# TruongKhang/cds-mvsnet

Measured on AMD Instinct MI355X. Metric: depth-maps/sec per ref view at 640x512 N=5 D=192 (single-stage plane sweep incl. CostRegNet + regression), higher is better.
Workload: dtype f32; 1 GPU; M1: single-stage StageNet volume 640x512, D=192, C=8, N=5 views; parallelism=single

## Files before the change

### cds_mvsnet_amd/_lib.py

```python
from __future__ import annotations

import ctypes
import os
from ctypes import c_float, c_int, c_longlong, c_void_p

_HERE = os.path.dirname(os.path.abspath(__file__))
LIB_PATH = os.environ.get("CDS_MVSNET_LIB") or os.path.join(_HERE, "libcdsmvs_hip.so")

ACT_NONE, ACT_RELU, ACT_LEAKY01, ACT_SIGMOID, ACT_TANH = 0, 1, 2, 3, 4
ACT_ACCUM = 16
AGG_ACCUMULATE, AGG_NORMALIZE, AGG_CHANNELS_LAST, AGG_FAST_POSITIONS = 1, 2, 4, 8
WARP_FAST_POSITIONS = AGG_FAST_POSITIONS
MAX_VIEWS = 8
MAX_IMAGES = 16
STAGE_STATE_WORDS = 2080
DEPTH_METRICS_MAX_T = 8
DEPTH_METRICS_MAX_GROUPS = 1024
ICP_SUMS = 18
ICP_MAX_GROUPS = 1024
CROP_MAX_VERTICES = 256
RANSAC_RECORD = 15
RANSAC_MIN_SAMPLE, RANSAC_MAX_SAMPLE = 3, 8
EINVAL = -1000

P = c_void_p
I = c_int
F = c_float
DB = ctypes.c_double
L = c_longlong

SIGNATURES = {
    "cds_version": [],
    "cds_chw_to_hwc_f32": [P, P, I, I, I, P],
    "cds_stage_inputs_f32": [P, P, P, P, P, P, P, P, P, P, I, I, I, I, P],
    "cds_homo_warp_f32": [P, P, P, P, I, I, I, I, I, P],
    "cds_warp_entropy_f32": [P, P, P, P, P, I, I, I, I, I, I, P],
    "cds_warp_entropy_flags_f32": [P, P, P, P, P, I, I, I, I, I, I, I, P],
    "cds_warp_aggregate_f32": [P, P, P, P, P, P, P, I, I, I, I, I, I, I, P],
    "cds_warp_entropy_window_f32": [P, P, P, P, P, I, I, I, I, I, I, I, I, P],
    "cds_warp_aggregate_window_f32": [P, P, P, P, P, P, P, I, I, I, I, I, I, I, I, P],
    "cds_warp_aggregate_bwd_f32": [P, P, P, P, P, P, P, P, P, I, I, I, I, I, I, P],
    "cds_volume_finish_f32": [P, P, P, I, I, I, I, P, P, P],
    "cds_volume_finish_bwd_f32": [P, P, P, P, P, I, I, I, I, P, P, P, P, P],
    "cds_volume_normalize_f32": [P, P, I, I, I, P],
    "cds_volume_normalize_cl_f32": [P, P, I, I, I, P],
    "cds_softargmin_conf_f32": [P, P, P, P, P, I, I, I, I, P],
    "cds_depth_hypotheses_f32": [P, P, I, I, I, I, I, I, P, P, P],
    "cds_depth_planes_f32": [P, I, I, I, P, P],
    "cds_conv3d_k3_f32": [P, P, P, P, P, I, I, I, I, I, I, I, P],
    "cds_conv3d_k3_cl_f32": [P, P, P, P, P, I, I, I, I, I, I, P],
    "cds_conv3d_sbf_f32": [P, P, P, P, P, I, I, I, I, I, I, I, P],
    "cds_conv3d_sf16_f32": [P, P, P, P, I, I, I, I, I, I, I, P, F, P, P],
    "cds_deconv3d_sbf_f32": [P, P, P, P, P, I, I, I, I, I, I, I, P],
    "cds_deconv3d_sf16_f32": [P, P, P, P, P, I, I, I, I, I, I, P, F, P, P],
    "cds_deconv3d_zm_sf16_f32": [P, P, P, P, P, I, I, I, I, I, I, P, F, P, P],
    "cds_deconv_prob_zm_f32": [P, P, P, P, P, P, I, I, I, P],
    "cds_deconv_prob_zm_sf16_f32": [P, P, P, P, P, P, I, I, I, P, F, P],
    "cds_deconv_prob_zm_sf16_mfma_f32": [P, P, P, P, P, P, P, I, I, I, P, F, P, F, F, P],
    "cds_deconv3d_zm_f32": [P, P, P, P, P, I, I, I, I, I, I, P],
    "cds_deconv3d_k3s2_f32": [P, P, P, P, P, I, I, I, I, I, I, P],
    "cds_conv2d_f32": [P, P, P, P, I, I, I, I, I, I, I, I, I, P],
    "cds_conv2d_affine_f32": [P, P, P, P, P, I, I, I, I, I, I, I, I, I, P],
    "cds_instnorm_affine_f32": [P, P, P, I, I, I, I, F, P],
    "cds_fpn_stats_parts": [I, I],
    "cds_conv2d_fpn_f32": [P, P, P, P, P, P, P, I, I, I, I, I, I, P],
    "cds_conv2d_k3_c16_f32": [P, P, P, P, P, P, I, I, I, I, P],
    "cds_dynconv_branches_sbf_f32": [P, P, P, P, P, I, I, I, I, I, P, I, P],
    "cds_dynconv_fused_sbf_f32": [P, P, P, P, P, P, P, P, F, P, P, P, I, I, I, I, I, P, I, P],
    "cds_dynconv_fused_parts": [I, I],
    "cds_conv2d_k3_relu_sbf_f32": [P, P, P, P, P, P, I, I, I, I, P],
    "cds_dynconv_blend_f32": [P, P, P, P, P, F, P, P, I, I, I, I, I, P],
    "cds_dynconv_blend_shared_f32": [P, P, P, P, P, F, P, P, I, I, I, I, I, I, P],
    "cds_blend_stats_parts": [I, I],
    "cds_dynconv_blend_stats_f32": [P, P, P, P, P, F, P, P, P, I, I, I, I, I, I, P],
    "cds_instnorm_reduce_f32": [P, I, P, P, I, I, I, I, F, P],
    "cds_instnorm_apply_f32": [P, P, P, I, I, I, I, I, I, P],
    "cds_instnorm_act_f32": [P, P, P, I, I, I, I, I, I, P],
    "cds_debug_poison_lds": [ctypes.c_uint],
    "cds_dynconv_cl_parts": [I, I],
    "cds_dynconv_cl_f32": [P, P, P, P, P, P, P, P, F, P, P, P, I, I, I, I, P, I, P],
    "cds_dynconv_cl_sf16_f32": [P, P, P, P, P, P, P, P, F, P, P, P, I, I, I, I, P, I, F, F, P],
    "cds_conv00_cl_f32": [P, P, P, P, P, P, P, F, P, P, P, I, I, I, I, P],
    "cds_conv00_cl_sf16_f32": [P, P, P, P, P, P, P, F, P, P, P, I, I, I, I, P, F, P],
    "cds_blend_cl_parts": [I, I],
    "cds_dynconv_blend_cl_f32": [P, P, P, P, P, F, P, P, P, I, I, I, I, I, I, P],
    "cds_conv2d_k3s2_cl_f32": [P, P, P, P, I, I, I, I, I, P],
    "cds_conv2d_k3s2_cl_sf16_f32": [P, P, P, P, I, I, I, I, I, F, F, P],
    "cds_fpn_cl_parts": [I, I],
    "cds_conv2d_fpn_cl_f32": [P, P, P, P, P, P, P, I, I, I, I, I, I, P],
    "cds_vis_layer1_cl_f32": [P, P, P, P, P, I, I, I, P],
    "cds_conv2d_k3_relu_cl_f32": [P, P, P, P, P, P, I, I, I, I, P],
    "cds_vis_cnn_rm_f32": [P, P, P, P, P, P, P, P, P, P, P, I, I, I, P],
    "cds_instnorm_stats_cl_parts": [I, I],
    "cds_instnorm_stats_cl_f32": [P, P, I, I, I, I, P],
    "cds_instnorm_apply_cl_f32": [P, P, P, P, I, I, I, I, I, I, I, P],
    "cds_curvature_stats_f32": [P, P, P, P, P, I, P],
    "cds_curvature_stats_bwd_f32": [P, P, P, P, P, P, P, P, I, P],
    "cds_pair_mean_f32": [P, P, I, I, P],
    "cds_view_mean_f32": [P, P, I, I, P],
    "cds_depth_affine_f32": [P, P, I, P, P],
    "cds_deconv2d_k3s2_f32": [P, P, P, P, I, I, I, I, I, P],
    "cds_refine_finish_f32": [P, P, P, I, I, P, P],
    "cds_bn3d_stats_f32": [P, P, I, I, L, P],
    "cds_bn3d_norm_f32": [P, P, P, P, DB, DB, F, P, P, P, P, P, P, P, P, I, I, L, I, P],
    "cds_bn3d_bwd_reduce_f32": [P, P, P, P, P, I, I, L, I, P],
    "cds_bn3d_bwd_norm_f32": [P, P, P, P, P, P, P, DB, P, P, P, I, I, L, I, P],
    "cds_conv3d_wgrad_f32": [P, P, P, I, I, I, I, I, I, I, I, I, I, P],
    "cds_bn3d_norm_bound_f32": [P, P, P, P, DB, DB, F, P, P, P, P, P, P, P, P, I, I, L, I, P, P],
    "cds_bn3d_bwd_norm_bound_f32": [P, P, P, P, P, P, P, DB, P, P, P, I, I, L, I, P, P],
    "cds_absmax_bound_f32": [P, L, P, P],
    "cds_sf16_pack_conv3d_f32": [P, P, P, P, I, I, I, P],
    "cds_conv3d_k3_sf16_f32": [P, P, P, P, P, I, I, I, I, I, I, I, P],
    "cds_conv3d_wgrad_sf16_f32": [P, P, P, P, P, I, I, I, I, I, I, I, I, I, I, P],
    "cds_conv2d_wgrad_f32": [P, P, P, I, I, I, I, I, I, I, I, I, I, P],
    "cds_conv2d_dgrad_s2_f32": [P, P, P, I, I, I, I, I, I, I, P],
    "cds_instnorm_bwd_f32": [P, P, P, P, P, I, I, I, I, I, I, P],
    "cds_dynconv_bn_stats_f32": [P, P, P, P, P, P, P, P, I, I, I, I, I, I, F, F, I, I, P],
    "cds_dynconv_blend_train_f32": [P, P, P, P, P, P, P, P, F, P, P, I, I, I, I, I, I, P],
    "cds_dynconv_blend_bwd_f32": [P, P, P, P, P, P, P, P, F, P, P, P, P, P, I, I, I, I, I, I, I, I, P],
    "cds_f32_to_bf16": [P, P, L, P],
    "cds_instnorm_act_b16_f32": [P, P, P, P, P, I, I, I, I, I, I, P],
    "cds_conv2d_wgrad_xb16_f32": [P, P, P, I, I, I, I, I, I, I, I, I, I, P],
    "cds_instnorm_bwd_yb16_f32": [P, P, P, P, P, P, I, I, I, I, I, I, P],
    "cds_dynconv_bn_stats_b16_f32": [P, P, P, P, P, P, P, P, I, I, I, I, I, I, F, F, I, I, P],
    "cds_dynconv_blend_train_b16_f32": [P, P, P, P, P, P, P, P, F, P, P, I, I, I, I, I, I, P],
    "cds_dynconv_blend_bwd_b16_f32": [P, P, P, P, P, P, P, P, F, P, P, P, P, P, I, I, I, I, I, I, I, I, P],
    "cds_pack_conv2d_f32": [P, P, P, P, I, I, I, I, P],
    "cds_pack_conv3d_f32": [P, P, P, I, I, I, P],
    "cds_softargmin_bwd_f32": [P, P, P, P, I, I, I, I, P],
    "cds_dynconv_bwd_finish_f32": [P, P, I, I, P, P],
    "cds_bn_running_update_f32": [P, P, P, F, I, I, P, P, P],
    "cds_loss_records": [ctypes.c_longlong],
    "cds_loss_stage_f32": [P, P, P, P, P, P, P, I, I, I, P, P, P],
    "cds_loss_final_f32": [P, P, P, P, P, P, I, P, P, P, P],
    "cds_loss_stage_bwd_f32": [P, P, P, P, P, P, P, P, F, I, I, I, P, P, P, P],
    "cds_feat_target_f32": [P, P, P, F, F, I, I, I, P, P],
    "cds_depth_fusion_f32": [P, P, P, P, P, P, P, P, P, I, I, I, P, F, F, F, P],
    "cds_depth_fusion_dynamic_f32": [P, P, P, P, P, P, P, P, P, P, I, I, I, P, F, F, I, I, P],
    "cds_depth_normals_f32": [P, P, P, I, I, I, F, I, P, P, P],
    "cds_voxel_merge_f32": [P, P, P, L, P, P, L, P, P, P, P, P],
    "cds_tsdf_integrate_f32": [P, L, P, P, DB, P, P, P, P, I, I, I, P, P, P, P, P],
    "cds_tsdf_integrate_w_f32": [P, L, P, P, DB, P, P, P, P, I, I, I, P, P, P, P, P, I, F, P, P],
    "cds_tsdf_view_weights": [P, P, P, P, P, P, I, I, P, P],
    "cds_tsdf_classify": [P, P, L, P, P, P, P, I, P, P, P, P, P],
    "cds_tsdf_emit": [P, P, L, P, P, P, P, P, P, P, P, P, P, L, L, P, P, P, P, P],
    "cds_raster_project": [P, L, P, I, P, P, P],
    "cds_raster_faces": [P, L, L, P, I, P, P, I, I, L, P, P, P],
    "cds_raster_large": [P, L, P, L, L, P, I, P, P, I, I, P, P],
    "cds_raster_resolve": [P, P, L, L, P, I, P, P, I, I, P, P, P, P, P, P],
    "cds_mesh_cc_init": [P, L, P],
    "cds_mesh_cc_hook": [P, L, L, P, P, P],
    "cds_mesh_cc_jump": [P, L, P],
    "cds_mesh_cc_count": [P, L, L, P, P, P],
    "cds_mesh_cc_mark": [P, L, L, P, P, P, P, P],
    "cds_mesh_cc_gather": [P, P, P, L, L, P, P, P, P, L, L, P, P, P, P],
    "cds_mesh_simplify_faces": [P, L, L, P, L, P, P, P, P],
    "cds_mesh_simplify_quadric_f32": [P, L, P, L, P, P, P, P, L, F, P, P, P],
    "cds_mesh_simplify_mark": [P, P, L, L, P, P],
    "cds_mesh_simplify_gather": [P, P, L, P, P, P, L, P, P, L, L, P, P, P, P],
    "cds_mesh_adj_small": [],
    "cds_mesh_adj_count": [P, L, L, P, P],
    "cds_mesh_adj_fill": [P, L, L, P, P, P, L, P],
    "cds_mesh_adj_finish": [L, P, P, L, P, P, P],
    "cds_mesh_smooth_step_f32": [P, P, L, P, P, P, DB, P],
    "cds_mesh_smooth_limit_f32": [P, P, L, DB, P, P, P],
    "cds_mesh_fill_max_edges": [],
    "cds_mesh_fill_keys": [P, L, L, P, P],
    "cds_mesh_fill_borders": [P, L, L, P, P, P, P, P],
    "cds_mesh_fill_init": [L, P, P, P, P, P, P, P, P, P, P],
    "cds_mesh_fill_double": [P, L, L, P, P, P, P, P],
    "cds_mesh_fill_walk": [P, P, L, P, P, P, P, L, I, P, P, P, P],
    "cds_mesh_fill_emit": [P, P, L, L, P, L, I, P, P, P, P, P, L, L, P, P, P, P],
    "cds_mesh_sample_max_n": [],
    "cds_mesh_sample_count": [P, L, P, L, DB, P, P, P],
    "cds_mesh_sample_emit": [P, P, L, P, L, P, P, L, P, P, P, P],
    "cds_texture_votes": [P, P, I, I, I, L, P, I, P],
    "cds_texture_best": [P, L, I, I, P, P],
    "cds_texture_cells": [P, L, P, L, P, I, P, L, DB, I, P, P, P],
    "cds_texture_place": [P, P, L, L, I, P, P, P],
    "cds_texture_fill": [P, P, L, P, L, P, P, L, P, I, P, P, P, P, L, I, I, I, P, I, P],
    "cds_texture_level_samples": [P, L, P, P, L, P, I, P, L, P, P, P],
    "cds_texture_level_pairs": [P, P, P, P, L, I, P, P],
    "cds_texture_level_step": [P, P, P, P, P, L, P, L, L, I, DB, P, P, P],
    "cds_texture_fill_level": [P, P, L, P, L, P, P, L, P, I, P, P, P, P, L, I, I, I, P, I, P, P, L, P],
    "cds_photo_shade": [P, L, P, L, P, P, I, I, P, I, P, I, I, P, P],
    "cds_photo_scores": [P, P, P, P, I, I, I, P, L, P, P, P, P],
    "cds_grid_hash_log2_slots": [L],
    "cds_grid_keys_f32": [P, L, P, P, P],
    "cds_grid_hash_build": [P, L, L, P, P, I, P],
    "cds_nn_query_f32": [P, P, L, P, P, P, P, P, P, I, P, F, P, P],
    "cds_thin_round_f32": [P, P, L, P, P, I, P, F, P, P, P],
    "cds_knn_mean_f64": [P, P, L, P, P, P, P, P, P, I, P, I, F, P, P, P],
    "cds_knn_mean_wg_f64": [P, P, L, P, P, P, P, P, P, I, P, I, F, P, P, I, P],
    "cds_radius_count_f32": [P, P, L, P, P, P, P, P, P, I, P, F, I, P, P],
    "cds_outlier_stats_f64": [P, L, P, L, P, P],
    "cds_transform_points_f32": [P, L, P, P, P],
    "cds_nn_index_f32": [P, P, L, P, P, P, P, P, P, I, P, F, P, P, P],
    "cds_icp_sums_f64": [P, P, L, P, P, P, P, P, P, P, I, P, F, P, L, P, P, P, P],
    "cds_voxel_mean_f32": [P, L, P, P, L, P, P],
    "cds_polygon_crop_f32": [P, L, P, I, I, DB, DB, P, P],
    "cds_ransac_similarity_f64": [P, P, L, L, I, DB, ctypes.c_ulonglong, P, L, P, P, P, P],
    "cds_gipuma_tiles": [L],
    "cds_gipuma_prob_filter_f32": [P, P, P, I, I, I, P, P, P, P],
    "cds_gipuma_fuse_view_f32": [P, P, P, P, I, I, I, I, F, F, F, I, P, P, P, P],
    "cds_gipuma_scan": [P, I, P, P, P, P],
    "cds_gipuma_compact_f32": [P, P, P, I, I, P, P, P, P],
    "cds_colmap_score_quantum_log2": [],
    "cds_colmap_score_limbs": [DB, DB, DB],
    "cds_colmap_pair_scores_f64": [P, P, P, P, P, P, L, L, I, DB, DB, DB, I, P, P],
    "cds_colmap_obs_depth_f64": [P, P, P, P, L, P, P],
    "cds_colmap_depth_ranges_f64": [P, P, P, P, I, P, P],
    "cds_depth_metrics_f32": [P, P, P, P, F, I, L, I, P, L, P, P],
    "cds_gt_pyramid_f32": [P, P, I, I, I, P, P, I, I, I, P, P, P],
    "cds_image_batch_u8": [P, I, I, I, P, P, I, I, P, P],
    "cds_eval_views_u8": [P, I, I, I, P, P, P, P, P, P, I, I, P, P],
    "cds_eval_outputs_f32": [P, I, I, P, I, I, P, I, I, P, I, I, P, I, I, P, P, P],
}

_lib = None


class CdsLibraryError(RuntimeError):
    pass


def load() -> ctypes.CDLL:
    global _lib
    if _lib is not None:
        return _lib
    if not os.path.exists(LIB_PATH):
        raise CdsLibraryError(
            f"{LIB_PATH} not found: build it with `make -C {os.path.join(_HERE, 'csrc')}` "
            "(or `python -c 'import __graft_entry__ as g; g.build()'`). "
            "cds_mvsnet_amd has no CPU / PyTorch fallback.")
    import torch

    lib = ctypes.CDLL(LIB_PATH)
    for name, argtypes in SIGNATURES.items():
        try:
            fn = getattr(lib, name)
        except AttributeError as e:
            raise CdsLibraryError(f"{LIB_PATH} does not export {name}") from e
        fn.argtypes = argtypes
        fn.restype = c_int
    _lib = lib
    return lib


def check(rc: int, what: str) -> None:
    if rc == 0:
        return
    if rc == EINVAL:
        raise ValueError(f"{what}: invalid argument (CDS_EINVAL)")
    raise RuntimeError(f"{what}: HIP error {-rc}")
```

### cds_mvsnet_amd/csrc/conv3d_zmg.hip

```cpp
#include <stdlib.h>

#include "cds_common.hpp"
#include "sbf_common.hpp"

namespace {

__device__ __attribute__((aligned(32))) float g_zmg_zeros[8];

struct ZGDefaults {
  static constexpr int S = 1, RD = 1, MB = 1, TXO = 16, TYO = 8, G = 1, NG = 1, CW = 8, RPW = 1, YS = 1, PF = 1;
  static constexpr bool PAIR = false, F16 = false, P32 = false;
};
template <class P>
struct ZgF16 : P {
  static constexpr bool F16 = true;
};

struct ZgPair8 : ZGDefaults {
  static constexpr bool PAIR = true;
  static constexpr int TXO = 32, G = 3;
};
struct ZgPair16 : ZGDefaults {
  static constexpr bool PAIR = true;
  static constexpr int RD = 2, TXO = 32, NG = 4, CW = 4;
};
struct ZgPair32 : ZGDefaults {
  static constexpr bool PAIR = true;
  static constexpr int RD = 4, TXO = 32, TYO = 3, NG = 3, CW = 4;
};
struct ZgConv1 : ZGDefaults {
  static constexpr int S = 2;
};
struct ZgConv2 : ZGDefaults {
  static constexpr int RD = 2, TXO = 32;
};
struct ZgConv3 : ZGDefaults {
  static constexpr int S = 2, RD = 2, MB = 2, TYO = 4;
};
struct ZgConv2F16 : ZgF16<ZgConv2> {
  static constexpr int RPW = 2;
  static constexpr bool P32 = true;
};
struct ZgConv3F16 : ZgF16<ZgConv3> {
  static constexpr int RPW = 2;
};
struct ZgConv4F16 : ZgF16<ZGDefaults> {
  static constexpr int RD = 4, MB = 2, TYO = 4, PF = 2;
};
struct ZgConv5F16 : ZgF16<ZGDefaults> {
  static constexpr int S = 2, RD = 4, MB = 4, TYO = 2, RPW = 2;
  static constexpr bool P32 = true;
};
struct ZgConv6F16 : ZgF16<ZGDefaults> {
  static constexpr int RD = 8, MB = 4, TYO = 2, RPW = 2, YS = 2;
};

template <class P>
struct ZG {
  static constexpr int S = P::S, RD = P::RD, MB = P::MB, TXO = P::TXO, TYO = P::TYO, G = P::G, NG = P::NG;
  static constexpr bool F16 = P::F16;
  static constexpr int NT = F16 ? 2 : 3;
  static constexpr bool PAIR = P::PAIR, DEINT = PAIR || S == 2;
  static constexpr int CW = P::CW, PW = 4, THREADS = (CW + PW) * 64;
  static constexpr int RPW = P::RPW, YS = P::YS, PF = P::PF;
  static_assert(PF == 1 || (PF == 2 && 2 * NG * NT <= 15), "operand prefetch distance (lgkmcnt is a 4-bit count)");
  static_assert(RD % RPW == 0 && MB % YS == 0, "rounds per wave / cout split");
  static constexpr int KSPL = RD / RPW, MBS = MB / YS;
  static_assert(CW % (KSPL * MBS) == 0 && (KSPL == 1 || KSPL == 2 || KSPL == 4), "consumer waves");
  static constexpr int PARTS = CW / (KSPL * MBS);
  static constexpr int ROWS = TYO / PARTS;
  static constexpr int XT = TXO / (PAIR ? 32 : 16);
  static constexpr int NTW = ROWS * XT * G;
  static_assert(TYO % PARTS == 0 && NTW % NG == 0 && (KSPL != 2 || NTW % 2 == 0), "tile split");
  static constexpr int KW = PAIR ? 4 : 3, KS = (9 * KW + 3) / 4;
  static constexpr int IX = (TXO - 1) * S + 3, IY = (TYO - 1) * S + 3;
  static constexpr int IXH = DEINT ? (IX + 1) / 2 : 0;
  static constexpr int IXP = DEINT ? 2 * IXH : IX;
  static constexpr bool P32 = P::P32;
  static_assert(!P32 || F16, "the 32-byte position holds two terms");
  static constexpr int PB = P32 ? 16 : POSB, TB = P32 ? IY * IXP * 16 : 16;
  static constexpr int SLICEB = IY * IXP * (P32 ? 32 : POSB), PLANEB = RD * SLICEB;
  static constexpr int NINIT = 3 - S;
  static constexpr int NRES = S * (G - 1) + 3, NNEW = S * G, R = NRES + NNEW;
  static constexpr int RINGB = R * PLANEB;
  static constexpr int XCH1 = KSPL == 2 ? CW * (NTW / 2) * 1024 : (KSPL == 4 ? CW * NTW * 1024 : 0);
  static constexpr int NFIN = KSPL == 4 ? (NTW + 3) / 4 : 1;
  static constexpr int tap_of(int t, int gg) {
    const int tap = PAIR ? 4 * t + ((gg & 1) * 2 + (gg >> 1)) : 4 * t + gg;
    return tap > 9 * KW - 1 ? 9 * KW - 1 : tap;
  }
  static constexpr int tap_kz(int t, int gg) { return tap_of(t, gg) / (3 * KW); }
  static constexpr int tap_off(int t, int gg) {
    const int tap = tap_of(t, gg), ky = (tap / KW) % 3, kx = tap % KW;
    return (ky * IXP + (DEINT ? ((kx & 1) * IXH + (kx >> 1)) : kx)) * PB;
  }
  static constexpr int LDSB = RINGB + 2 * XCH1;
  static_assert(LDSB <= 160 * 1024, "LDS budget");
  static constexpr int NITEM = NNEW * IY * RD * IXP;
  static constexpr int PT = PW * 64, PPT = (NITEM + PT - 1) / PT;
};

template <class Cfg>
__global__ __launch_bounds__(Cfg::THREADS, 1) void conv3d_zmg_kernel(const float* __restrict__ x, const uint4* __restrict__ wsp,
                                                                  const float* __restrict__ bias, float* __restrict__ out, int Cout,
                                                                  int D, int H, int W, int Do, int Ho, int Wo, int act,
                                                                  int tiles_x, int tiles_y, int zseg,
                                                                  const float* __restrict__ in_bound, float w_inv,
                                                                  float* __restrict__ out_bound) {
  constexpr int S = Cfg::S, RD = Cfg::RD, G = Cfg::G, R = Cfg::R, Cin = 8 * RD, KS = Cfg::KS, NTW = Cfg::NTW, NG = Cfg::NG;
  constexpr bool PAIR = Cfg::PAIR, F16 = Cfg::F16;
  constexpr int NT = Cfg::NT;
  const float xs = F16 ? sf16_scale(in_bound[0]) : 1.0f;
  const float out_mul = F16 ? w_inv / xs : 1.0f;
  extern __shared__ __attribute__((aligned(16))) unsigned char lds[];
  const int tid = threadIdx.x;
  const int lane = tid & 63;
  const int wave = __builtin_amdgcn_readfirstlane(tid >> 6);
  const int nseg = (Do + zseg - 1) / zseg;
  int unit = cds_xcd_remap(blockIdx.x, gridDim.x);
  const int seg = unit % nseg;
  unit /= nseg;
  const int tx_i = unit % tiles_x, ty_i = unit / tiles_x;
  const int z0 = seg * zseg, z1 = min(Do, z0 + zseg);
  const int nstages = (z1 - z0 + G - 1) / G;
  const int gx0 = tx_i * Cfg::TXO * S - 1, gy0 = ty_i * Cfg::TYO * S - 1;
  const int zin0 = S * z0 - 1;

  if (wave >= Cfg::CW) {
#ifndef CDS_ZMG_PPRIO
#define CDS_ZMG_PPRIO 3
#endif
    __builtin_amdgcn_s_setprio(CDS_ZMG_PPRIO);
    constexpr int PT = Cfg::PT, PPT = Cfg::PPT;
    const int ptid = tid - Cfg::CW * 64;
    int s_pl[PPT], s_dst[PPT];
    long long s_off[PPT];
    unsigned okmask = 0;
#pragma unroll
    for (int h = 0; h < PPT; ++h) {
      const int p = h * PT + ptid;
      const int q = p % Cfg::IXP, t1 = p / Cfg::IXP;
      const int rd = t1 % RD, t2 = t1 / RD;
      const int row = t2 % Cfg::IY, pl = t2 / Cfg::IY;
      const int c = Cfg::DEINT ? (2 * (q % Cfg::IXH) + q / Cfg::IXH) : q;
      const int gy = gy0 + row, gx = gx0 + c;
      const bool exists = p < Cfg::NITEM && c < Cfg::IX;
      s_pl[h] = pl;
      s_dst[h] = rd * Cfg::SLICEB + (row * Cfg::IXP + q) * Cfg::PB;
      s_off[h] = ((long long)gy * W + gx) * Cin + rd * 8;
      if (exists && (unsigned)gy < (unsigned)H && (unsigned)gx < (unsigned)W) okmask |= 1u << h;
      if (!exists) s_pl[h] = -1;
    }
    const long long plane_elems = (long long)H * W * Cin;
    float4 va[2][PPT], vb[2][PPT];
    auto issue = [&](int st, int set) {
      const int zn = zin0 + st * S * G + Cfg::NINIT;
#pragma unroll
      for (int h = 0; h < PPT; ++h) {
        const int z = zn + s_pl[h];
        const bool ok = ((okmask >> h) & 1u) && (unsigned)z < (unsigned)D;
        const float* __restrict__ src = ok ? x + ((long long)z * plane_elems + s_off[h]) : g_zmg_zeros;
        va[set][h] = *reinterpret_cast<const float4*>(src);
        vb[set][h] = *reinterpret_cast<const float4*>(src + 4);
      }
    };
    auto deposit = [&](int st, int set) {
      const int slot0 = (st * S * G + Cfg::NINIT) % R;
#pragma unroll
      for (int h = 0; h < PPT; ++h) {
        if (h + 1 == PPT && s_pl[h] < 0) continue;
        int slot = slot0 + (s_pl[h] < 0 ? 0 : s_pl[h]);
        slot = slot >= R ? slot - R : slot;
        if (Cfg::P32) split_store8_f16_planar(lds + slot * Cfg::PLANEB + s_dst[h], Cfg::TB, va[set][h], vb[set][h], xs);
        else if (F16) split_store8_f16(lds + slot * Cfg::PLANEB + s_dst[h], va[set][h], vb[set][h], xs);
        else split_store8(lds + slot * Cfg::PLANEB + s_dst[h], va[set][h], vb[set][h]);
      }
    };
    for (int p = ptid; p < Cfg::NINIT * Cfg::IY * RD * Cfg::IXP; p += PT) {
      const int q = p % Cfg::IXP, t1 = p / Cfg::IXP;
      const int rd = t1 % RD, t2 = t1 / RD;
      const int row = t2 % Cfg::IY, pl = t2 / Cfg::IY;
      const int c = Cfg::DEINT ? (2 * (q % Cfg::IXH) + q / Cfg::IXH) : q;
      const int gz = zin0 + pl, gy = gy0 + row, gx = gx0 + c;
      const bool ok = c < Cfg::IX && (unsigned)gz < (unsigned)D && (unsigned)gy < (unsigned)H && (unsigned)gx < (unsigned)W;
      const float* __restrict__ src = ok ? x + (((long long)gz * H + gy) * W + gx) * Cin + rd * 8 : g_zmg_zeros;
      unsigned char* dst = lds + pl * Cfg::PLANEB + rd * Cfg::SLICEB + (row * Cfg::IXP + q) * Cfg::PB;
      if (Cfg::P32) split_store8_f16_planar(dst, Cfg::TB, *reinterpret_cast<const float4*>(src), *reinterpret_cast<const float4*>(src + 4), xs);
      else if (F16) split_store8_f16(dst, *reinterpret_cast<const float4*>(src), *reinterpret_cast<const float4*>(src + 4), xs);
      else split_store8(dst, *reinterpret_cast<const float4*>(src), *reinterpret_cast<const float4*>(src + 4));
    }
    issue(0, 0);
    if (nstages > 1) issue(1, 1);
    deposit(0, 0);
    if (nstages > 2) issue(2, 0);
    __syncthreads();
    for (int st = 0; st < nstages; st += 2) {
      if (st + 1 < nstages) {
        deposit(st + 1, 1);
        if (st + 3 < nstages) issue(st + 3, 1);
      }
      __syncthreads();
      if (st + 1 >= nstages) break;
      if (st + 2 < nstages) {
        deposit(st + 2, 0);
        if (st + 4 < nstages) issue(st + 4, 0);
      }
      __syncthreads();
    }
    return;
  }

#ifndef CDS_ZMG_CPRIO
#define CDS_ZMG_CPRIO 2
#endif
  __builtin_amdgcn_s_setprio(CDS_ZMG_CPRIO);
  const int k = wave % Cfg::KSPL, mbi = (wave / Cfg::KSPL) % Cfg::MBS, part = wave / (Cfg::KSPL * Cfg::MBS);
  const int j = lane & 15, g = lane >> 4;
#ifdef CDS_ZMG_NOSKEW
  const bool late = false;
#else
  const bool late = Cfg::CW == 8 && wave >= 4;
#endif
  const int lane_base = k * Cfg::RPW * Cfg::SLICEB + (part * Cfg::ROWS * S * Cfg::IXP + j) * Cfg::PB +
                        (PAIR ? (((g & 1) * 2 + (g >> 1)) & 1) * Cfg::IXH * Cfg::PB + ((((g & 1) * 2 + (g >> 1))) >> 1) * Cfg::PB : 0);
  constexpr int RPW = Cfg::RPW;
  const int mbg = (Cfg::YS > 1 ? blockIdx.y * Cfg::MBS : 0) + mbi;
  BV wres[RPW * KS][NT];
  {
    const uint4* __restrict__ wl = wsp + lane;
#pragma unroll
    for (int t = 0; t < RPW * KS; ++t) {
      const size_t o = (size_t)(((k * RPW * KS + t) * Cfg::MB + mbg) * 3) * 64;
#pragma unroll
      for (int tm = 0; tm < NT; ++tm) wres[t][tm].u = wl[o + 64 * tm];
    }
  }
  float amax = 0.f;
  const int co = PAIR ? 4 * (g & 1) : mbg * 16 + 4 * g;
  const float4 bv = (bias && co < Cout) ? *reinterpret_cast<const float4*>(bias + co) : make_float4(0.f, 0.f, 0.f, 0.f);
  constexpr int XW = PAIR ? 32 : 16;
  const int oy0 = ty_i * Cfg::TYO + part * Cfg::ROWS;
  const int ox0 = tx_i * Cfg::TXO + (PAIR ? 2 * j + (g >> 1) : j);
  float* const obase = out + ((size_t)((size_t)z0 * Ho + oy0) * Wo + ox0) * Cout + co;
  float* const obase_u = out + ((size_t)((size_t)z0 * Ho + oy0) * Wo + tx_i * Cfg::TXO) * Cout;
  const unsigned olane = (unsigned)((ox0 - tx_i * Cfg::TXO) * Cout + co);
  auto out_ptr = [&](int pl, int r, int xt) -> float* {
    const size_t o = ((size_t)((size_t)pl * Ho + r) * Wo + xt * XW) * Cout;
    return Cfg::P32 ? obase_u + o + olane : obase + o;
  };
  bool lane_ok[Cfg::XT];
#pragma unroll
  for (int xt = 0; xt < Cfg::XT; ++xt) lane_ok[xt] = ox0 + xt * XW < Wo && co < Cout;
  auto in_x_ct = [&](int xt) { return lane_ok[xt]; };
  auto in_x_rt = [&](int xt) { return ox0 + xt * XW < Wo && co < Cout; };
  auto store_tile = [&](int n, int st, const f32x4& a, auto in_x) {
    const int i = n % G, rx = n / G, xt = rx % Cfg::XT, r = rx / Cfg::XT;
    if (z0 + st * G + i >= z1 || oy0 + r >= Ho) return;
    if (!in_x(xt)) return;
    float4 o = F16 ? sf16_rescale4(a, out_mul, bv) : sbf_add4(sbf_f4(a), bv);
    if (act == CDS_ACT_RELU) o = sbf_relu4(o);
    if (F16) amax = sbf_amax4(amax, o);
    sbf_store4(out_ptr(st * G + i, r, xt), o);
  };
  unsigned char* xch = lds + Cfg::RINGB;
  constexpr int NH = NTW / 2;
  f32x4 acc[NTW];
  constexpr bool KEEP4 = Cfg::RPW == 1;
  f32x4 keep[Cfg::KSPL == 2 ? NH : Cfg::NFIN];
  const int xgrp = (wave / Cfg::KSPL) * NTW;
  auto finish = [&](int sp) {
    if (Cfg::KSPL == 2) {
      const unsigned char* src = xch + (sp & 1) * Cfg::XCH1 + ((wave ^ 1) * NH) * 1024 + lane * 16;
#pragma unroll
      for (int m = 0; m < NH; ++m) {
        const f32x4 o = *reinterpret_cast<const f32x4*>(src + m * 1024);
        store_tile(k * NH + m, sp, k == 0 ? keep[m] + o : o + keep[m], in_x_ct);
      }
    } else if (Cfg::KSPL == 4) {
#pragma unroll
      for (int jf = 0; jf < Cfg::NFIN; ++jf) {
        const int n = jf * 4 + k;
        if (n >= NTW) continue;
        const unsigned char* src = xch + (sp & 1) * Cfg::XCH1 + ((xgrp + n) * 4) * 1024 + lane * 16;
        f32x4 total = KEEP4 && k == 0 ? keep[jf] : *reinterpret_cast<const f32x4*>(src);
#pragma unroll
        for (int kk = 1; kk < 4; ++kk) total = total + (KEEP4 && kk == k ? keep[jf] : *reinterpret_cast<const f32x4*>(src + kk * 1024));
        store_tile(n, sp, total, in_x_rt);
      }
    } else {
#pragma unroll
      for (int n = 0; n < NTW; ++n) store_tile(n, sp, acc[n], in_x_ct);
    }
  };
  __syncthreads();
  for (int st = 0; st < nstages; ++st) {
    if (late && st > 0) finish(st - 1);
    int vpl[PAIR ? Cfg::NRES : 1];
    int vaddr[PAIR ? 1 : KS][PAIR ? 1 : G];
    {
      int sl[Cfg::NRES];
      int slot = (st * S * G) % R;
#pragma unroll
      for (int u = 0; u < Cfg::NRES; ++u) {
        sl[u] = slot * Cfg::PLANEB;
        slot = slot + 1 >= R ? slot + 1 - R : slot + 1;
      }
      if (PAIR) {
#pragma unroll
        for (int u = 0; u < Cfg::NRES; ++u) vpl[u] = lane_base + sl[u];
      } else {
#pragma unroll
        for (int t = 0; t < KS; ++t)
#pragma unroll
          for (int i = 0; i < G; ++i) {
            const int o0 = sl[S * i + Cfg::tap_kz(t, 0)] + Cfg::tap_off(t, 0), o1 = sl[S * i + Cfg::tap_kz(t, 1)] + Cfg::tap_off(t, 1);
            const int o2 = sl[S * i + Cfg::tap_kz(t, 2)] + Cfg::tap_off(t, 2), o3 = sl[S * i + Cfg::tap_kz(t, 3)] + Cfg::tap_off(t, 3);
            vaddr[t][i] = lane_base + (g == 0 ? o0 : (g == 1 ? o1 : (g == 2 ? o2 : o3)));
          }
      }
    }
    constexpr int NGRP = NTW / NG, NS = RPW * KS * NGRP;
    constexpr int PF = Cfg::PF;
    BV bd[PF + 1][NG][NT];
    auto load_b = [&](int buf, int ss) {
      const int t = (ss / NGRP) % KS, rr = ss / (NGRP * KS), grp = ss % NGRP;
#pragma unroll
      for (int q = 0; q < NG; ++q) {
        const int n = grp * NG + q, i = n % G, rx = n / G, xt = rx % Cfg::XT, r = rx / Cfg::XT;
        const unsigned char* b = lds + (PAIR ? vpl[PAIR ? S * i + t / 3 : 0] + (t % 3) * Cfg::IXP * Cfg::PB : vaddr[PAIR ? 0 : t][PAIR ? 0 : i]) +
                                 (r * S * Cfg::IXP + xt * 16) * Cfg::PB + rr * Cfg::SLICEB;
        bd[buf][q][0].u = *reinterpret_cast<const uint4*>(b);
        bd[buf][q][1].u = *reinterpret_cast<const uint4*>(b + Cfg::TB);
        if (!F16) bd[buf][q][NT - 1].u = *reinterpret_cast<const uint4*>(b + 32);
      }
    };
    load_b(0, 0);
    if (PF == 2 && NS > 1) load_b(1, 1);
    __builtin_amdgcn_s_setprio(0);
#pragma unroll
    for (int t = 0; t < NTW; ++t) acc[t] = (f32x4){0.f, 0.f, 0.f, 0.f};
#pragma unroll
    for (int ss = 0; ss < NS; ++ss) {
      const int t = ss / NGRP, grp = ss % NGRP, db = ss % (PF + 1);
      if (ss + PF < NS) load_b((ss + PF) % (PF + 1), ss + PF);
      __builtin_amdgcn_sched_barrier(0);
#ifndef CDS_ZMG_LAZYWAIT
      if (ss + PF < NS) __builtin_amdgcn_s_waitcnt(0xC07F | ((PF * NT * NG) << 8));
      else if (PF == 2 && ss + 1 < NS) __builtin_amdgcn_s_waitcnt(0xC07F | ((NT * NG) << 8));
      else __builtin_amdgcn_s_waitcnt(0xC07F);
      __builtin_amdgcn_sched_barrier(0);
#endif
      if constexpr (F16) {
        SF16_TERMS(acc, grp * NG, NG, wres[t], bd[db]);
      } else {
        SBF_TERMS(acc, grp * NG, NG, wres[t], bd[db]);
      }
    }
    __builtin_amdgcn_s_setprio(CDS_ZMG_CPRIO);
    if (Cfg::KSPL == 2) {
      if (!late && st > 0) finish(st - 1);
      unsigned char* dst = xch + (st & 1) * Cfg::XCH1 + (wave * NH) * 1024 + lane * 16;
#pragma unroll
      for (int m = 0; m < NH; ++m) {
        *reinterpret_cast<f32x4*>(dst + m * 1024) = acc[(k ^ 1) * NH + m];
        keep[m] = acc[k * NH + m];
      }
    } else if (Cfg::KSPL == 4) {
      if (!late && st > 0) finish(st - 1);
      unsigned char* dst = xch + (st & 1) * Cfg::XCH1 + (xgrp * 4 + k) * 1024 + lane * 16;
#pragma unroll
      for (int n = 0; n < NTW; ++n) {
        if (KEEP4 && (n & 3) == k) keep[n >> 2] = acc[n];
        else *reinterpret_cast<f32x4*>(dst + n * 4096) = acc[n];
      }
    } else if (!late) {
      finish(st);
    }
    __syncthreads();
  }
  if (Cfg::KSPL >= 2 || late) finish(nstages - 1);
  if (F16) sf16_publish_bound(amax, out_bound);
}

inline int zmg_pick_nseg(int cols, int Do, int G) {
  const int nseg_env = cds_env_int("CDS_ZMG_NSEG", 0);
  if (nseg_env > 0) return nseg_env;
  const int stages = cds_ceil_div(Do, G);
  int best = 1;
  double best_cost = 1e30;
  for (int n = 1; n <= 32 && n <= stages; ++n) {
    const int per = cds_ceil_div(stages, n);
    if (n > 1 && per < 6) break;
    const double cost = (double)cds_ceil_div(cols * cds_ceil_div(stages, per), 256) * (per + 2.5);
    if (cost < best_cost - 1e-9) { best_cost = cost; best = n; }
  }
  return best;
}

template <class P>
int launch_zmg(const float* x, const void* wsp, const float* b, float* out, int Cout, int D, int H, int W, int act, hipStream_t st,
               const float* in_bound = nullptr, float w_inv = 1.f, float* out_bound = nullptr, int min_wgs = 0) {
  using Cfg = ZG<P>;
  constexpr int S = Cfg::S;
  const int Do = (D - 1) / S + 1, Ho = (H - 1) / S + 1, Wo = (W - 1) / S + 1;
  const int tx = cds_ceil_div(Wo, Cfg::TXO), ty = cds_ceil_div(Ho, Cfg::TYO);
  int nseg = zmg_pick_nseg(tx * ty * Cfg::YS, Do, Cfg::G);
  const int zseg = cds_ceil_div(cds_ceil_div(Do, nseg), Cfg::G) * Cfg::G;
  nseg = cds_ceil_div(Do, zseg);
  if (min_wgs > 0 && tx * ty * nseg * Cfg::YS < min_wgs) return CDS_ZMG_UNSUPPORTED;
  return cds_launch_lds<conv3d_zmg_kernel<Cfg>>(Cfg::LDSB, dim3(tx * ty * nseg, Cfg::YS), dim3(Cfg::THREADS), Cfg::LDSB, st, x,
                                                reinterpret_cast<const uint4*>(wsp), b, out, Cout, D, H, W, Do, Ho, Wo, act, tx, ty, zseg,
                                                in_bound, w_inv, out_bound);
}

}

int cds_conv3d_zmg_dispatch(const float* x, const void* wsp, const float* bias, float* out, int Cin, int Cout, int D, int H, int W,
                            int stride, int pair, int act, hipStream_t st, const float* in_bound, float w_inv, float* out_bound) {
  const bool f16 = in_bound != nullptr;
  auto off = [] { return cds_env_is("CDS_ZMG", '0'); };
  if (!f16 && off()) return CDS_ZMG_UNSUPPORTED;
  auto run = [&](auto p, int min_wgs = 0) {
    return launch_zmg<decltype(p)>(x, wsp, bias, out, Cout, D, H, W, act, st, in_bound, w_inv, out_bound, min_wgs);
  };
  if (pair) {
    if (Cin == 8) return f16 ? run(ZgF16<ZgPair8>()) : run(ZgPair8());
    if (Cin == 16) return f16 ? run(ZgF16<ZgPair16>()) : run(ZgPair16());
    if (Cin == 32) return f16 ? run(ZgF16<ZgPair32>()) : run(ZgPair32());
    return CDS_ZMG_UNSUPPORTED;
  }
  if (stride == 2 && Cin == 8 && Cout == 16) return f16 ? run(ZgF16<ZgConv1>()) : run(ZgConv1());
  if (stride == 1 && Cin == 16 && Cout == 16) return f16 ? run(ZgConv2F16()) : run(ZgConv2());
  if (stride == 2 && Cin == 16 && Cout == 32) return f16 ? run(ZgConv3F16()) : run(ZgConv3());
  if (!f16) return CDS_ZMG_UNSUPPORTED;
  const int deep = off() ? 0 : cds_env_int("CDS_ZMG_DEEP", 1);
  const int min_wgs = deep == 2 ? 0 : 256;
  if (deep <= 0) return CDS_ZMG_UNSUPPORTED;
  if (stride == 1 && Cin == 32 && Cout == 32) return run(ZgConv4F16(), min_wgs);
  if (stride == 2 && Cin == 32 && Cout == 64) return run(ZgConv5F16(), min_wgs);
  if (stride == 1 && Cin == 64 && Cout == 64) return run(ZgConv6F16(), min_wgs);
  return CDS_ZMG_UNSUPPORTED;
}
```

### cds_mvsnet_amd/csrc/deconv3d_zm.hip

```cpp
#include "zm_common.hpp"

namespace {

template <int ROUNDS_, int TY_ = 8>
struct DZC {
  static constexpr int ROUNDS = ROUNDS_;
  static constexpr int TX = 16, TY = TY_;
  static constexpr int IX = TX + 1, IY = TY + 1, IXP = 18;
  static constexpr int ROUNDB = IY * IXP * POSB;
  static constexpr int SLOTB = ROUNDS * ROUNDB;
  static constexpr int NSLOT = 3;
  static constexpr int CW = 8, PW = 4, THREADS = (CW + PW) * 64;
  static constexpr int LDS = NSLOT * SLOTB;
  static constexpr int NITEM = IY * IX * ROUNDS;
};

template <class C, bool F16>
__device__ __forceinline__ void dzm_produce(const float* __restrict__ x, unsigned char* lds, int ptid, int X0, int Y0, int D, int H, int W,
                                            int a0, int a1, float xs) {
  __builtin_amdgcn_s_setprio(3);
  ZmCellStage<C, C::PW * 64, F16, false> stage;
  stage.init(ptid, X0, Y0, H, W);
  auto issue = [&](int plane) { stage.issue(x, plane, D, H, W); };
  auto deposit = [&](int plane) { stage.deposit(lds + (plane % C::NSLOT) * C::SLOTB, xs); };
  issue(a0);
  deposit(a0);
  issue(a0 + 1);
  deposit(a0 + 1);
  issue(a0 + 2);
  __syncthreads();
  for (int a = a0; a < a1; ++a) {
    deposit(a + 2);
    issue(a + 3);
    __syncthreads();
  }
}

template <int ROUNDS, bool F16>
__global__ __launch_bounds__((DZC<ROUNDS>::THREADS), 3) void deconv3d_zm_kernel(
    const float* __restrict__ x, const uint4* __restrict__ wcls, const float* __restrict__ bias, const float* __restrict__ skip,
    float* __restrict__ out, int D, int H, int W, int tiles_x, int ncols, int seg_len, int act, const float* __restrict__ in_bound,
    float w_inv, float* __restrict__ out_bound) {
  using C = DZC<ROUNDS>;
  constexpr int NT = F16 ? 2 : 3;
  const float xs = F16 ? sf16_scale(in_bound[0]) : 1.0f;
  const float out_mul = F16 ? w_inv / xs : 1.0f;
  constexpr int Cout = 16;
  extern __shared__ __attribute__((aligned(16))) unsigned char lds[];
  const int tid = threadIdx.x;
  const int lane = tid & 63;
  const int wave = __builtin_amdgcn_readfirstlane(tid >> 6);
  const ZmColumn zc = zm_column(tiles_x, ncols, seg_len, D);
  const int a0 = zc.a0, a1 = zc.a1;
  if (a0 >= a1) return;
  const int X0 = zc.tx_i * C::TX, Y0 = zc.ty_i * C::TY;
  const int Ho = 2 * H, Wo = 2 * W;

  if (wave >= C::CW) {
    dzm_produce<C, F16>(x, lds, tid - C::CW * 64, X0, Y0, D, H, W, a0, a1, xs);
    return;
  }

  const int pz = wave >> 2, py = (wave >> 1) & 1, px = wave & 1;
  if (pz) __builtin_amdgcn_s_setprio(1);
  const int j = lane & 15, g = lane >> 4;
  BV wlo[ROUNDS][3], whi[ROUNDS][3];
  {
    const uint4* __restrict__ wp = wcls + (size_t)wave * ROUNDS * 2 * 3 * 64 + lane;
#pragma unroll
    for (int rd = 0; rd < ROUNDS; ++rd)
#pragma unroll
      for (int k = 0; k < NT; ++k) {
        wlo[rd][k].u = wp[((rd * 2 + 0) * 3 + k) * 64];
        whi[rd][k].u = wp[((rd * 2 + 1) * 3 + k) * 64];
      }
  }
  const float4 bv = bias ? *reinterpret_cast<const float4*>(bias + 4 * g) : make_float4(0.f, 0.f, 0.f, 0.f);
  const int b_off = (((g >> 1) * C::IXP) + j + (g & 1)) * POSB;
  const int xv = 2 * (X0 + j) + px;
  const bool x_ok = X0 + j < W;
  const size_t zstride = (size_t)Ho * Wo * Cout;
  float amax = 0.f;
  __syncthreads();
  for (int a = a0; a < a1; ++a) {
    const unsigned char* lo = lds + (a % C::NSLOT) * C::SLOTB + b_off;
    const unsigned char* hi = lds + ((a + 1) % C::NSLOT) * C::SLOTB + b_off;
    const size_t zbase = (size_t)(2 * a + pz) * zstride;
    const int nrows = min(C::TY, H - Y0);
    float4 skn = make_float4(0.f, 0.f, 0.f, 0.f);
    auto row_off = [&](int n) { return ((size_t)(2 * (Y0 + n) + py) * Wo + xv) * Cout + 4 * g; };
    if (skip && x_ok) skn = *reinterpret_cast<const float4*>(skip + zbase + row_off(0));
    asm volatile("" ::"v"(skn.x), "v"(skn.y), "v"(skn.z), "v"(skn.w));
    for (int n = 0; n < nrows; ++n) {
      const float4 sk = skn;
      if (skip && x_ok && n + 1 < nrows) skn = *reinterpret_cast<const float4*>(skip + zbase + row_off(n + 1));
      f32x4 acc[1] = {F16 ? (f32x4){0.f, 0.f, 0.f, 0.f} : (f32x4){bv.x, bv.y, bv.z, bv.w}};
      const unsigned char* lo_n = lo + n * C::IXP * POSB;
      const unsigned char* hi_n = hi + n * C::IXP * POSB;
#pragma unroll
      for (int rd = 0; rd < ROUNDS; ++rd) {
        BV b[1][3];
        b[0][0].u = *reinterpret_cast<const uint4*>(lo_n + rd * C::ROUNDB);
        b[0][1].u = *reinterpret_cast<const uint4*>(lo_n + rd * C::ROUNDB + 16);
        if constexpr (F16) {
          SF16_TERMS(acc, 0, 1, wlo[rd], b);
        } else {
          b[0][2].u = *reinterpret_cast<const uint4*>(lo_n + rd * C::ROUNDB + 32);
          SBF_TERMS(acc, 0, 1, wlo[rd], b);
        }
        if (pz) {
          BV c[1][3];
          c[0][0].u = *reinterpret_cast<const uint4*>(hi_n + rd * C::ROUNDB);
          c[0][1].u = *reinterpret_cast<const uint4*>(hi_n + rd * C::ROUNDB + 16);
          if constexpr (F16) {
            SF16_TERMS(acc, 0, 1, whi[rd], c);
          } else {
            c[0][2].u = *reinterpret_cast<const uint4*>(hi_n + rd * C::ROUNDB + 32);
            SBF_TERMS(acc, 0, 1, whi[rd], c);
          }
        }
      }
      asm volatile("" ::"v"(skn.x), "v"(skn.y), "v"(skn.z), "v"(skn.w));
      if (x_ok) {
        float4 o = F16 ? sf16_rescale4(acc[0], out_mul, bv) : sbf_f4(acc[0]);
        if (act == CDS_ACT_RELU) o = sbf_relu4(o);
        if (skip) o = sbf_add4(sk, o);
        if (F16) amax = sbf_amax4(amax, o);
        sbf_store4(out + zbase + row_off(n), o);
      }
    }
    __syncthreads();
  }
  if (F16) sf16_publish_bound(amax, out_bound);
}


constexpr int DZM64_W1L = 2;
__global__ __launch_bounds__((DZC<8, 4>::THREADS), 3) void deconv3d_zm64_kernel(
    const float* __restrict__ x, const uint4* __restrict__ wsp, const float* __restrict__ bias, const float* __restrict__ skip,
    float* __restrict__ out, int D, int H, int W, int tiles_x, int ncols, int seg_len, int act, const float* __restrict__ in_bound,
    float w_inv, float* __restrict__ out_bound) {
  using C = DZC<8, 4>;
  constexpr int ROUNDS = 8, Cout = 32, NKS = 9, W1L = DZM64_W1L;
  const float xs = sf16_scale(in_bound[0]);
  const float out_mul = w_inv / xs;
  extern __shared__ __attribute__((aligned(16))) unsigned char lds[];
  const int tid = threadIdx.x;
  const int lane = tid & 63;
  const int wave = __builtin_amdgcn_readfirstlane(tid >> 6);
  const ZmColumn zc = zm_column(tiles_x, ncols, seg_len, D);
  const int a0 = zc.a0, a1 = zc.a1;
  if (a0 >= a1) return;
  const int mbtot = gridDim.y, mb0 = blockIdx.y;
  const int X0 = zc.tx_i * C::TX, Y0 = zc.ty_i * C::TY;
  const int Ho = 2 * H, Wo = 2 * W;

  if (wave >= C::CW) {
    dzm_produce<C, true>(x, lds, tid - C::CW * 64, X0, Y0, D, H, W, a0, a1, xs);
    return;
  }

  const int pz = wave >> 2, py = (wave >> 1) & 1, px = wave & 1;
  const bool two = wave == 7;
  if (two) __builtin_amdgcn_s_setprio(1);
  const int j = lane & 15, g = lane >> 4;
  BV w0[ROUNDS][2], w1[ROUNDS - W1L][2];
  unsigned char* w1l = lds + C::LDS + lane * 16;
  {
    const uint4* __restrict__ wp = wsp + lane;
#pragma unroll
    for (int rd = 0; rd < ROUNDS; ++rd)
#pragma unroll
      for (int k = 0; k < 2; ++k) {
        w0[rd][k].u = wp[(size_t)(((rd * NKS + wave) * mbtot + mb0) * 3 + k) * 64];
        const uint4 v = wp[(size_t)(((rd * NKS + (two ? 8 : wave)) * mbtot + mb0) * 3 + k) * 64];
        if (rd < ROUNDS - W1L) w1[rd][k].u = v;
        else if (two) *reinterpret_cast<uint4*>(w1l + ((rd - (ROUNDS - W1L)) * 2 + k) * 1024) = v;
      }
  }
  const float4 bv = bias ? *reinterpret_cast<const float4*>(bias + mb0 * 16 + 4 * g) : make_float4(0.f, 0.f, 0.f, 0.f);
  const int ny = 1 + py, nx = 1 + px;
  const bool live = g < (1 + pz) * ny * nx;
  const int dz = live ? g / (ny * nx) : 0, dy = live ? (g / nx) % ny : 0, dx = live ? g % nx : 0;
  const int b_off = ((dy * C::IXP) + j + dx) * POSB;
  const int xv = 2 * (X0 + j) + px;
  const bool x_ok = X0 + j < W;
  const size_t zstride = (size_t)Ho * Wo * Cout;
  const int nrows = min(C::TY, H - Y0);
  float amax = 0.f;
  __syncthreads();
  for (int a = a0; a < a1; ++a) {
    const unsigned char* p0 = lds + (a % C::NSLOT) * C::SLOTB + b_off;
    const unsigned char* hi = lds + ((a + 1) % C::NSLOT) * C::SLOTB + b_off;
    const unsigned char* lo = dz ? hi : p0;
    const size_t zbase = (size_t)(2 * a + pz) * zstride;
    float4 skn = make_float4(0.f, 0.f, 0.f, 0.f);
    auto row_off = [&](int n) { return ((size_t)(2 * (Y0 + n) + py) * Wo + xv) * Cout + mb0 * 16 + 4 * g; };
    if (skip && x_ok) skn = *reinterpret_cast<const float4*>(skip + zbase + row_off(0));
    asm volatile("" ::"v"(skn.x), "v"(skn.y), "v"(skn.z), "v"(skn.w));
    for (int n = 0; n < nrows; ++n) {
      const float4 sk = skn;
      if (skip && x_ok && n + 1 < nrows) skn = *reinterpret_cast<const float4*>(skip + zbase + row_off(n + 1));
      f32x4 acc[1] = {(f32x4){0.f, 0.f, 0.f, 0.f}};
      const unsigned char* lo_n = lo + n * C::IXP * POSB;
      const unsigned char* hi_n = hi + n * C::IXP * POSB;
#pragma unroll
      for (int rd = 0; rd < ROUNDS; ++rd) {
        BV b[1][2];
        b[0][0].u = *reinterpret_cast<const uint4*>(lo_n + rd * C::ROUNDB);
        b[0][1].u = *reinterpret_cast<const uint4*>(lo_n + rd * C::ROUNDB + 16);
        SF16_TERMS(acc, 0, 1, w0[rd], b);
        if (two) {
          BV c[1][2];
          c[0][0].u = *reinterpret_cast<const uint4*>(hi_n + rd * C::ROUNDB);
          c[0][1].u = *reinterpret_cast<const uint4*>(hi_n + rd * C::ROUNDB + 16);
          if (rd < ROUNDS - W1L) {
            SF16_TERMS(acc, 0, 1, w1[rd < ROUNDS - W1L ? rd : 0], c);
          } else {
            BV wl[2];
            wl[0].u = *reinterpret_cast<const uint4*>(w1l + ((rd - (ROUNDS - W1L)) * 2 + 0) * 1024);
            wl[1].u = *reinterpret_cast<const uint4*>(w1l + ((rd - (ROUNDS - W1L)) * 2 + 1) * 1024);
            SF16_TERMS(acc, 0, 1, wl, c);
          }
        }
      }
      asm volatile("" ::"v"(skn.x), "v"(skn.y), "v"(skn.z), "v"(skn.w));
      if (x_ok) {
        float4 o = sf16_rescale4(acc[0], out_mul, bv);
        if (act == CDS_ACT_RELU) o = sbf_relu4(o);
        if (skip) o = sbf_add4(sk, o);
        amax = sbf_amax4(amax, o);
        sbf_store4(out + zbase + row_off(n), o);
      }
    }
    __syncthreads();
  }
  sf16_publish_bound(amax, out_bound);
}

}

int cds_deconv3d_zm64_dispatch(const float* x, const void* wsp, const float* bias, const float* skip, float* out, int Cin, int Cout,
                               int D, int H, int W, int act, hipStream_t st, const float* in_bound, float w_inv, float* out_bound) {
  const int deep = cds_env_int("CDS_DZM_DEEP", 1);
  if (deep <= 0 || Cin != 64 || Cout != 32 || !in_bound) return CDS_ZMG_UNSUPPORTED;
  if ((long)2 * H * 2 * W * Cout >= (1l << 31) || (long)H * W * Cin >= (1l << 31)) return CDS_ZMG_UNSUPPORTED;
  using C = DZC<8, 4>;
  const int tiles_x = cds_ceil_div(W, C::TX), tiles_y = cds_ceil_div(H, C::TY);
  const int ncols = tiles_x * tiles_y;
  const int seg_len = cds_ceil_div(D, zm_pick_nseg(ncols * 2, D, 24, "CDS_DZM_NSEG"));
  const int nseg = cds_ceil_div(D, seg_len);
  if (deep == 1 && ncols * nseg * 2 < 256) return CDS_ZMG_UNSUPPORTED;
  return cds_launch_lds<deconv3d_zm64_kernel>(160 * 1024, dim3(ncols * nseg, 2), dim3(C::THREADS), C::LDS + DZM64_W1L * 2 * 1024, st, x,
                                              reinterpret_cast<const uint4*>(wsp), bias, skip, out, D, H, W, tiles_x, ncols, seg_len, act,
                                              in_bound, w_inv, out_bound);
}

static int dzm_entry(const float* x, const void* weight_cls, const float* bias, const float* skip, float* out, int Cin, int Cout, int D,
                     int H, int W, int act, const float* in_bound, float w_inv, float* out_bound, void* stream) {
  if (!x || !weight_cls || !out || Cin != 32 || Cout != 16 || D < 1 || H < 1 || W < 1) return CDS_EINVAL;
  if ((long)2 * H * 2 * W * Cout >= (1l << 31) || (long)H * W * Cin >= (1l << 31)) return CDS_EINVAL;
  using C = DZC<4>;
  hipStream_t st = (hipStream_t)stream;
  const int tiles_x = cds_ceil_div(W, C::TX), tiles_y = cds_ceil_div(H, C::TY);
  const int ncols = tiles_x * tiles_y;
  const int seg_len = cds_ceil_div(D, zm_pick_nseg(ncols, D, 24, "CDS_DZM_NSEG"));
  const int nseg = cds_ceil_div(D, seg_len);
  auto launch = [&](auto f16) {
    return cds_launch_lds<deconv3d_zm_kernel<4, decltype(f16)::value>>(160 * 1024, dim3(ncols * nseg), dim3(C::THREADS), C::LDS, st, x,
                                                                       reinterpret_cast<const uint4*>(weight_cls), bias, skip, out, D, H, W,
                                                                       tiles_x, ncols, seg_len, act, in_bound, w_inv, out_bound);
  };
  return in_bound ? launch(std::true_type()) : launch(std::false_type());
}

extern "C" int cds_deconv3d_zm_f32(const float* x, const void* weight_cls, const float* bias, const float* skip, float* out,
                                   int Cin, int Cout, int D, int H, int W, int act, void* stream) {
  return dzm_entry(x, weight_cls, bias, skip, out, Cin, Cout, D, H, W, act, nullptr, 1.0f, nullptr, stream);
}

extern "C" int cds_deconv3d_zm_sf16_f32(const float* x, const void* weight_cls, const float* bias, const float* skip, float* out,
                                        int Cin, int Cout, int D, int H, int W, int act, const float* in_bound, float w_inv_scale,
                                        float* out_bound, void* stream) {
  if (!in_bound || !(w_inv_scale > 0.f)) return CDS_EINVAL;
  return dzm_entry(x, weight_cls, bias, skip, out, Cin, Cout, D, H, W, act, in_bound, w_inv_scale, out_bound, stream);
}
```

### cds_mvsnet_amd/csrc/deconv_prob_zm.hip

```cpp
#include "zm_common.hpp"

namespace {

struct DPZ {
  static constexpr int CXC = 32, CYC = 8;
  static constexpr int CXR = CXC - 2, CYR = CYC - 2;
  static constexpr int NT = CXC / 16;
  static constexpr int IY = CYC + 1, IX = CXC + 1, IXP = 34;
  static constexpr int ROUNDS = 2;
  static constexpr int ROUNDB = IY * IXP * POSB;
  static constexpr int SLOTB = ROUNDS * ROUNDB;
  static constexpr int NA = 5;
  static constexpr int WB = ROUNDS * NA * 3 * 1024;
  static constexpr int YX = 2 * CXC, YY = 2 * CYC;
  static constexpr int YHALFB = YX * 16, YROWB = 2 * YHALFB;
  static constexpr int YB = YY * YROWB;
  static constexpr int CW = CYC, PW = 4, THREADS = (CW + PW) * 64;
  static constexpr int LDS = WB + 2 * SLOTB + 2 * YB;
  static constexpr int PR = 3;
  static constexpr int NITEM = IY * IX * ROUNDS;
  static constexpr int MT = 5, MSTEP = 12;
  static constexpr int YTERMB = YROWB / 2, YPARB = YTERMB / 2;
};
static_assert(DPZ::MT * DPZ::MSTEP == 2 * DPZ::CXR && (DPZ::MT - 1) * DPZ::MSTEP + 16 <= DPZ::YX, "prob x tiles");
static_assert(DPZ::PW * DPZ::PR == 2 * DPZ::CYR, "prob rows");
static_assert(DPZ::LDS <= 160 * 1024, "LDS budget");

__device__ __forceinline__ float dpz_fma(float d, float w, float acc) {
  asm("v_fmac_f32 %0, %1, %2" : "+v"(acc) : "s"(w), "v"(d));
  return acc;
}

__device__ __forceinline__ float dpz_row_shr1(float v) {
  return __int_as_float(__builtin_amdgcn_update_dpp(0, __float_as_int(v), 0x111, 0xF, 0xF, true));
}
__device__ __forceinline__ float dpz_row_shl1(float v) {
  return __int_as_float(__builtin_amdgcn_update_dpp(0, __float_as_int(v), 0x101, 0xF, 0xF, true));
}

#define DPZ_TERMS(ACC, W, X)                                  \
  do {                                                        \
    if constexpr (F16) { SF16_TERMS(ACC, 0, C::NT, W, X); }   \
    else { SBF_TERMS(ACC, 0, C::NT, W, X); }                  \
  } while (0)
template <bool F16, bool MF>
__global__ __launch_bounds__(DPZ::THREADS, 3) void deconv_prob_zm_kernel(
    const float* __restrict__ x, const uint4* __restrict__ wsp, const float* __restrict__ bias, const float* __restrict__ skip,
    const float* __restrict__ pw, float* __restrict__ out, int D, int H, int W, int tiles_x, int ncols, int seg_len,
    const float* __restrict__ in_bound, float w_inv, const float* __restrict__ skip_bound, float y_gain, float p_inv) {
  static_assert(F16 || !MF, "the matrix-core prob form exists in split-f16 only");
  using C = DPZ;
  const float xs = F16 ? sf16_scale(in_bound[0]) : 1.0f;
  const float out_mul = F16 ? w_inv / xs : 1.0f;
  float ys = 1.0f;
  if constexpr (MF) {
    float bmax = 0.f;
    for (int i = 0; i < 8; ++i) bmax = fmaxf(bmax, fabsf(bias[i]));
    ys = sf16_scale(skip_bound[0] + y_gain * in_bound[0] + bmax);
  }
  extern __shared__ __attribute__((aligned(16))) unsigned char lds[];
  unsigned char* const inring = lds + C::WB;
  unsigned char* const ybuf = inring + 2 * C::SLOTB;
  const int tid = threadIdx.x;
  const int lane = tid & 63;
  const int wave = __builtin_amdgcn_readfirstlane(tid >> 6);
  const ZmColumn zc = zm_column(tiles_x, ncols, seg_len, D);
  const int tx_i = zc.tx_i, ty_i = zc.ty_i, a0 = zc.a0, a1 = zc.a1;
  if (a0 >= a1) return;
  const int X0 = tx_i * C::CXR - 1, Y0 = ty_i * C::CYR - 1;
  const int Do = 2 * D, Ho = 2 * H, Wo = 2 * W;
  const int qs = a0 > 0 ? 2 * a0 - 1 : 0;
  const int qe = min(Do - 1, 2 * a1);
  const int te = 2 * a1 + 1;
  {
    uint4* wdst = reinterpret_cast<uint4*>(lds);
    for (int i = tid; i < C::WB / 16; i += C::THREADS) wdst[i] = wsp[i];
  }

  if (wave >= C::CW) {
    __builtin_amdgcn_s_setprio(2);
    const int ptid = tid - C::CW * 64;
    ZmCellStage<C, C::PW * 64, F16, true> stage;
    stage.init(ptid, X0, Y0, H, W);
    auto issue = [&](int plane) { stage.issue(x, plane, D, H, W); };
    auto deposit = [&](int plane) { stage.deposit(inring + (plane & 1) * C::SLOTB, xs); };
    if constexpr (MF) {
      const int n = lane & 15, g = lane >> 4, rg = wave - C::CW;
      const uint4* __restrict__ pwm = reinterpret_cast<const uint4*>(pw);
      BV wa[3][3];
#pragma unroll
      for (int r = 0; r < 3; ++r)
#pragma unroll
        for (int ky = 0; ky < 3; ++ky) wa[r][ky].u = pwm[(r * 3 + ky) * 64 + lane];
      const int oy0 = ty_i * 2 * C::CYR + C::PR * rg;
      int b_off[C::MT];
#pragma unroll
      for (int t = 0; t < C::MT; ++t) {
        const int xl = C::MSTEP * t + n;
        b_off[t] = (g & 1) * C::YTERMB + (xl & 1) * C::YPARB + (((xl >> 1) ^ ((xl & 1) << 3)) << 4);
      }
      const int ox0 = tx_i * 2 * C::CXR + n - 2;
      const bool st_ok = g < 3 && n >= 2 && n <= 13;
      const unsigned st_lane = st_ok ? oy0 * Wo + ox0 : 0;
      const int st_lim = st_ok ? Wo - ox0 : 0;
      const float inv = p_inv / ys;
      float A[C::MT][C::PR];
#pragma unroll
      for (int t = 0; t < C::MT; ++t)
#pragma unroll
        for (int r = 0; r < C::PR; ++r) A[t][r] = 0.f;
      const int yrow0 = (C::PR * rg + 1) * C::YROWB;
      auto load_b = [&](BV (&b)[C::PR + 2], const unsigned char* yb, int t) {
#pragma unroll
        for (int rho = 0; rho < C::PR + 2; ++rho) b[rho].u = *reinterpret_cast<const uint4*>(yb + rho * C::YROWB + b_off[t]);
      };
      auto process = [&](int q, auto rc) {
        constexpr int R = decltype(rc)::value;
        const unsigned char* yb = ybuf + (q & 1) * C::YB + yrow0;
        BV b[2][C::PR + 2];
        load_b(b[0], yb, 0);
#pragma unroll
        for (int t = 0; t < C::MT; ++t) {
          if (t + 1 < C::MT) load_b(b[(t + 1) & 1], yb, t + 1);
          f32x4 d[C::PR];
#pragma unroll
          for (int r = 0; r < C::PR; ++r) {
            d[r] = (f32x4){0.f, 0.f, 0.f, 0.f};
#pragma unroll
            for (int ky = 0; ky < 3; ++ky) SF16_MFMA(d[r], wa[R][ky], b[t & 1][r + ky]);
          }
#pragma unroll
          for (int r = 0; r < C::PR; ++r) {
            float s = d[r][1] + dpz_row_shr1(d[r][0]);
            s = s + dpz_row_shl1(d[r][2]);
            A[t][r] = A[t][r] + s;
          }
        }
      };
      const int ap = qs >> 1;
      issue(ap);
      deposit(ap);
      if (qs & 1) {
        issue(ap + 1);
        deposit(ap + 1);
      }
      __syncthreads();
      for (int t = qs; t <= te; ++t) {
        const int q = t - 1;
        if (q >= qs && q <= qe) {
          const int R = (q + 1) % 3;
          if (R == 0) process(q, std::integral_constant<int, 0>());
          else if (R == 1) process(q, std::integral_constant<int, 1>());
          else process(q, std::integral_constant<int, 2>());
        }
        const int o = t - 2;
        const bool own = g == (3 - (o + 3) % 3) % 3;
        if (o >= 2 * a0 && o < 2 * a1) {
          float* po = out + (size_t)o * Ho * Wo;
#pragma unroll
          for (int r = 0; r < C::PR; ++r)
            if (oy0 + r < Ho) {
#pragma unroll
              for (int tt = 0; tt < C::MT; ++tt)
                if (own && C::MSTEP * tt < st_lim) (po + r * Wo + C::MSTEP * tt)[st_lane] = A[tt][r] * inv;
            }
        }
#pragma unroll
        for (int tt = 0; tt < C::MT; ++tt)
#pragma unroll
          for (int r = 0; r < C::PR; ++r) A[tt][r] = own ? 0.f : A[tt][r];
        __syncthreads();
      }
      return;
    }
    const int c = ptid & 63, rg = ptid >> 6;
    const int ox = tx_i * 2 * C::CXR + c;
    const int oy0 = ty_i * 2 * C::CYR + C::PR * rg;
    const bool lane_ok = c < 2 * C::CXR && ox < Wo;
    const int yoff = (C::PR * rg + 1) * C::YROWB + (c + 1) * 16;
    int st_off[C::PR];
#pragma unroll
    for (int r = 0; r < C::PR; ++r) st_off[r] = (lane_ok && oy0 + r < Ho) ? (oy0 + r) * Wo + ox : -1;
    float A[3][C::PR];
#pragma unroll
    for (int s = 0; s < 3; ++s)
#pragma unroll
      for (int r = 0; r < C::PR; ++r) A[s][r] = 0.f;
    const f32x4* __restrict__ pw4 = reinterpret_cast<const f32x4*>(pw);
    auto load_d = [&](f32x4 (&d)[C::PR + 2], const unsigned char* yb, int b) {
#pragma unroll
      for (int rho = 0; rho < C::PR + 2; ++rho)
        d[rho] = *reinterpret_cast<const f32x4*>(yb + rho * C::YROWB + (b & 1) * C::YHALFB + (b >> 1) * 16);
    };
    auto load_w = [&](f32x4 (&w)[9], int b) {
#pragma unroll
      for (int k = 0; k < 9; ++k) w[k] = pw4[b * 9 + k];
    };
    auto compute = [&](const f32x4 (&d)[C::PR + 2], const f32x4 (&w)[9]) {
#pragma unroll
      for (int ky = 0; ky < 3; ++ky)
#pragma unroll
        for (int kz = 0; kz < 3; ++kz) {
          const f32x4 wv = w[ky * 3 + kz];
#pragma unroll
          for (int r = 0; r < C::PR; ++r) {
            const f32x4 dv = d[r + ky];
            float acc = A[2 - kz][r];
            acc = dpz_fma(dv.x, wv.x, acc);
            acc = dpz_fma(dv.y, wv.y, acc);
            acc = dpz_fma(dv.z, wv.z, acc);
            acc = dpz_fma(dv.w, wv.w, acc);
            A[2 - kz][r] = acc;
          }
        }
    };
    f32x4 wq0[9], wq1[9];
    load_w(wq0, 0);
    auto process = [&](int q) {
      const unsigned char* yb = ybuf + (q & 1) * C::YB + yoff;
      f32x4 d0[C::PR + 2], d1[C::PR + 2];
      load_d(d0, yb, 0);
#define DPZ_BATCH(B, DC, WC, DN, WN)                                   \
      __builtin_amdgcn_s_waitcnt(0xC07F);     \
      __builtin_amdgcn_sched_barrier(0);                               \
      load_w(WN, ((B) + 1) % 6);                                       \
      if ((B) + 1 < 6) load_d(DN, yb, (B) + 1);                        \
      __builtin_amdgcn_sched_barrier(0);                               \
      compute(DC, WC);                                                 \
      __builtin_amdgcn_sched_barrier(0);
      DPZ_BATCH(0, d0, wq0, d1, wq1)
      DPZ_BATCH(1, d1, wq1, d0, wq0)
      DPZ_BATCH(2, d0, wq0, d1, wq1)
      DPZ_BATCH(3, d1, wq1, d0, wq0)
      DPZ_BATCH(4, d0, wq0, d1, wq1)
      DPZ_BATCH(5, d1, wq1, d0, wq0)
#undef DPZ_BATCH
    };
    const int ap = qs >> 1;
    issue(ap);
    deposit(ap);
    if (qs & 1) {
      issue(ap + 1);
      deposit(ap + 1);
    }
    __syncthreads();
    for (int t = qs; t <= te; ++t) {
      const int q = t - 1;
      if (q >= qs && q <= qe) process(q);
      const int o = t - 2;
      if (o >= 2 * a0 && o < 2 * a1) {
        float* po = out + (size_t)o * Ho * Wo;
#pragma unroll
        for (int r = 0; r < C::PR; ++r)
          if (st_off[r] >= 0) po[st_off[r]] = A[0][r];
      }
#pragma unroll
      for (int r = 0; r < C::PR; ++r) {
        A[0][r] = A[1][r];
        A[1][r] = A[2][r];
        A[2][r] = 0.f;
      }
      __syncthreads();
    }
    return;
  }

  const int j = lane & 15, g = lane >> 4;
  const int px = g >> 1, co = 4 * (g & 1);
  const float4 bv = *reinterpret_cast<const float4*>(bias + co);
  const unsigned char* const wl = lds + lane * 16;
  const int b_h1 = ((wave + (g >> 1)) * C::IXP + j + (g & 1)) * POSB;
  const int b_h2a = (wave * C::IXP + j + (g & 1)) * POSB;
  const int b_h2b = b_h2a + C::IXP * POSB;
  int sk_off[2][C::NT];
#pragma unroll
  for (int py = 0; py < 2; ++py)
#pragma unroll
    for (int q = 0; q < C::NT; ++q) {
      const int xv = 2 * (X0 + 16 * q + j) + px, yv = 2 * (Y0 + wave) + py;
      sk_off[py][q] = (xv >= 0 && xv < Wo && yv >= 0 && yv < Ho) ? (yv * Wo + xv) * 8 + co : -1;
    }
  const bool border = X0 < 0 || X0 + C::CXC > W || Y0 < 0 || Y0 + C::CYC > H;
  const int y_off = MF ? (2 * wave) * C::YROWB + px * C::YPARB + ((j ^ (px << 3)) << 4) + (g & 1) * 8
                       : (2 * wave) * C::YROWB + (g & 1) * C::YHALFB + (2 * j + px) * 16;
  const size_t zstride = (size_t)Ho * Wo * 8;
  float4 sk0[2][C::NT], sk1[2][C::NT];
  auto load_skip = [&](float4 (&sk)[2][C::NT], int t) {
    if (t > qe) return;
    const float* __restrict__ sp = skip + (size_t)t * zstride;
#pragma unroll
    for (int py = 0; py < 2; ++py)
#pragma unroll
      for (int q = 0; q < C::NT; ++q) {
        const int o = sk_off[py][q];
        const float4 v = *reinterpret_cast<const float4*>(sp + max(o, 0));
        sk[py][q] = o >= 0 ? v : make_float4(0.f, 0.f, 0.f, 0.f);
      }
  };
  auto load_a = [&](BV (&wa)[3], int rd, int k) {
    const unsigned char* p = wl + (rd * C::NA + k) * 3 * 1024;
    wa[0].u = *reinterpret_cast<const uint4*>(p);
    wa[1].u = *reinterpret_cast<const uint4*>(p + 1024);
    if (!F16) wa[2].u = *reinterpret_cast<const uint4*>(p + 2048);
  };
  auto load_b = [&](BV (&bd)[C::NT][3], const unsigned char* p) {
#pragma unroll
    for (int q = 0; q < C::NT; ++q) {
      bd[q][0].u = *reinterpret_cast<const uint4*>(p + q * 16 * POSB);
      bd[q][1].u = *reinterpret_cast<const uint4*>(p + q * 16 * POSB + 16);
      if (!F16) bd[q][2].u = *reinterpret_cast<const uint4*>(p + q * 16 * POSB + 32);
    }
  };
  f32x4 acc[2][C::NT];
  auto epilogue = [&](const float4 (&sk)[2][C::NT], int par) {
    unsigned char* yb = ybuf + par * C::YB + y_off;
#pragma unroll
    for (int py = 0; py < 2; ++py)
#pragma unroll
      for (int q = 0; q < C::NT; ++q) {
        f32x4 a = acc[py][q];
        if (F16) a = a * out_mul + (f32x4){bv.x, bv.y, bv.z, bv.w};
        float4 o = sbf_add4(sk[py][q], sbf_relu4(sbf_f4(a)));
        if (border && sk_off[py][q] < 0) o = make_float4(0.f, 0.f, 0.f, 0.f);
        if constexpr (MF) {
          uint32_t h0, l0, h1, l1;
          split2_f16(o.x, o.y, ys, h0, l0);
          split2_f16(o.z, o.w, ys, h1, l1);
          unsigned char* yp = yb + py * C::YROWB + q * 16 * 16;
          *reinterpret_cast<uint2*>(yp) = make_uint2(h0, h1);
          *reinterpret_cast<uint2*>(yp + C::YTERMB) = make_uint2(l0, l1);
        } else {
          *reinterpret_cast<float4*>(yb + py * C::YROWB + q * 32 * 16) = o;
        }
      }
  };
  ZmCellStage<C, C::CW * 64, F16, true> stage;
  stage.init(tid, X0, Y0, H, W);
  if (qs & 1) load_skip(sk1, qs); else load_skip(sk0, qs);
  __syncthreads();
  for (int t = qs; t <= te; ++t) {
    if (t <= qe) {
      const int a = t >> 1;
      const unsigned char* cur = inring + (a & 1) * C::SLOTB;
#pragma unroll
      for (int py = 0; py < 2; ++py)
#pragma unroll
        for (int q = 0; q < C::NT; ++q)
          acc[py][q] = F16 ? (f32x4){0.f, 0.f, 0.f, 0.f} : (f32x4){bv.x, bv.y, bv.z, bv.w};
      if (!(t & 1)) {
        stage.issue(x, a + 1, D, H, W);
        load_skip(sk1, t + 1);
        BV w0[3], w1[3], b0[C::NT][3], b1[C::NT][3];
        load_b(b0, cur + b_h1);
        load_a(w0, 0, 0);
        load_a(w1, 0, 1);
        load_b(b1, cur + C::ROUNDB + b_h1);
        __builtin_amdgcn_sched_barrier(0);
        DPZ_TERMS(acc[0], w0, b0);
        load_a(w0, 1, 0);
        __builtin_amdgcn_sched_barrier(0);
        DPZ_TERMS(acc[1], w1, b0);
        load_a(w1, 1, 1);
        __builtin_amdgcn_sched_barrier(0);
        DPZ_TERMS(acc[0], w0, b1);
        DPZ_TERMS(acc[1], w1, b1);
        epilogue(sk0, 0);
        stage.deposit(inring + ((a + 1) & 1) * C::SLOTB, xs);
      } else {
        load_skip(sk0, t + 1);
        const unsigned char* oth = inring + ((a + 1) & 1) * C::SLOTB;
        const unsigned char* bz = (g >> 1) ? oth : cur;
        BV w0[3], w1[3], b0[C::NT][3], b1[C::NT][3];
#pragma unroll
        for (int rd = 0; rd < C::ROUNDS; ++rd) {
          load_b(b0, bz + rd * C::ROUNDB + b_h2a);
          load_a(w0, rd, 2);
          load_a(w1, rd, 3);
          load_b(b1, bz + rd * C::ROUNDB + b_h2b);
          __builtin_amdgcn_sched_barrier(0);
          DPZ_TERMS(acc[0], w0, b0);
          load_a(w0, rd, 4);
          __builtin_amdgcn_sched_barrier(0);
          DPZ_TERMS(acc[1], w1, b0);
          DPZ_TERMS(acc[1], w0, b1);
        }
        epilogue(sk1, 1);
      }
    }
    __syncthreads();
  }
}

}

static int dpz_entry(const float* x, const void* weight_split, const float* bias, const float* skip, const float* prob_table, float* out,
                     int D, int H, int W, const float* in_bound, float w_inv, void* stream, const float* skip_bound = nullptr,
                     float y_gain = 0.f, float p_inv = 1.f) {
  if (!x || !weight_split || !bias || !skip || !prob_table || !out || D < 1 || H < 1 || W < 1) return CDS_EINVAL;
  if ((long)2 * H * 2 * W * 8 >= (1l << 31) || (long)H * W * 16 >= (1l << 31)) return CDS_EINVAL;
  using C = DPZ;
  hipStream_t st = (hipStream_t)stream;
  const int tiles_x = cds_ceil_div(W, C::CXR), tiles_y = cds_ceil_div(H, C::CYR);
  const int ncols = tiles_x * tiles_y;
  const int seg_len = cds_ceil_div(D, zm_pick_nseg(ncols, D, 16, "CDS_DPZ_NSEG"));
  const int nseg = cds_ceil_div(D, seg_len);
  auto launch = [&](auto f16, auto mf) {
    return cds_launch_lds<deconv_prob_zm_kernel<decltype(f16)::value, decltype(mf)::value>>(
        160 * 1024, dim3(ncols * nseg), dim3(C::THREADS), C::LDS, st, x, reinterpret_cast<const uint4*>(weight_split), bias, skip, prob_table,
        out, D, H, W, tiles_x, ncols, seg_len, in_bound, w_inv, skip_bound, y_gain, p_inv);
  };
  if (skip_bound) return launch(std::true_type(), std::true_type());
  return in_bound ? launch(std::true_type(), std::false_type()) : launch(std::false_type(), std::false_type());
}

extern "C" int cds_deconv_prob_zm_f32(const float* x, const void* weight_split, const float* bias, const float* skip,
                                      const float* prob_table, float* out, int D, int H, int W, void* stream) {
  return dpz_entry(x, weight_split, bias, skip, prob_table, out, D, H, W, nullptr, 1.0f, stream);
}

extern "C" int cds_deconv_prob_zm_sf16_f32(const float* x, const void* weight_split, const float* bias, const float* skip,
                                           const float* prob_table, float* out, int D, int H, int W, const float* in_bound,
                                           float w_inv_scale, void* stream) {
  if (!in_bound || !(w_inv_scale > 0.f)) return CDS_EINVAL;
  return dpz_entry(x, weight_split, bias, skip, prob_table, out, D, H, W, in_bound, w_inv_scale, stream);
}

extern "C" int cds_deconv_prob_zm_sf16_mfma_f32(const float* x, const void* weight_split, const float* bias, const float* skip,
                                                const float* prob_table, const void* prob_mfma, float* out, int D, int H, int W,
                                                const float* in_bound, float w_inv_scale, const float* skip_bound, float y_gain,
                                                float p_inv_scale, void* stream) {
  if (!in_bound || !(w_inv_scale > 0.f) || !prob_mfma || !skip_bound || !(y_gain >= 0.f) || !(p_inv_scale > 0.f)) return CDS_EINVAL;
  const char* e = getenv("CDS_DPZ_PROB_MFMA");
  if (e && atoi(e) == 0) return dpz_entry(x, weight_split, bias, skip, prob_table, out, D, H, W, in_bound, w_inv_scale, stream);
  return dpz_entry(x, weight_split, bias, skip, static_cast<const float*>(prob_mfma), out, D, H, W, in_bound, w_inv_scale, stream,
                   skip_bound, y_gain, p_inv_scale);
}
```

### cds_mvsnet_amd/csrc/zm_common.hpp

```cpp
#pragma once
#include "sbf_common.hpp"

namespace {

struct ZmColumn {
  int tx_i, ty_i, a0, a1;
};
__device__ __forceinline__ ZmColumn zm_column(int tiles_x, int ncols, int seg_len, int D) {
  const int wg = cds_xcd_remap(blockIdx.x, gridDim.x);
  const int col = wg % ncols, seg = wg / ncols;
  const int a0 = seg * seg_len;
  return {col % tiles_x, col / tiles_x, a0, min(D, a0 + seg_len)};
}

template <class C, int NTHR, bool F16, bool LOWHALO>
struct ZmCellStage {
  static constexpr int Cin = 8 * C::ROUNDS;
  static constexpr int IPT = (C::NITEM + NTHR - 1) / NTHR;
  int src[IPT], dst[IPT];
  float4 va[IPT], vb[IPT];

  __device__ __forceinline__ void init(int t, int X0, int Y0, int H, int W) {
#pragma unroll
    for (int h = 0; h < IPT; ++h) {
      const int it = h * NTHR + t;
      const int rd = it % C::ROUNDS, p = it / C::ROUNDS;
      const int row = p / C::IX, c = p - row * C::IX;
      const int gy = Y0 + row, gx = X0 + c;
      const bool ok = it < C::NITEM && (!LOWHALO || gy >= 0) && gy < H && (!LOWHALO || gx >= 0) && gx < W;
      src[h] = ok ? ((gy * W + gx) * Cin + rd * 8) : -1;
      dst[h] = it < C::NITEM ? rd * C::ROUNDB + (row * C::IXP + c) * POSB : -1;
    }
  }
  __device__ __forceinline__ void issue(const float* __restrict__ x, int plane, int D, int H, int W) {
    const bool pok = plane < D;
    const float* __restrict__ xp = x + (size_t)min(plane, D - 1) * H * W * Cin;
#pragma unroll
    for (int h = 0; h < IPT; ++h) {
      const bool ok = pok && src[h] >= 0;
      const float* s = xp + (ok ? src[h] : 0);
      const float4 a = *reinterpret_cast<const float4*>(s), b = *reinterpret_cast<const float4*>(s + 4);
      va[h] = ok ? a : make_float4(0.f, 0.f, 0.f, 0.f);
      vb[h] = ok ? b : make_float4(0.f, 0.f, 0.f, 0.f);
    }
  }
  __device__ __forceinline__ void deposit(unsigned char* slot, float xs) const {
#pragma unroll
    for (int h = 0; h < IPT; ++h)
      if (dst[h] >= 0) {
        if (F16) split_store8_f16(slot + dst[h], va[h], vb[h], xs);
        else split_store8(slot + dst[h], va[h], vb[h]);
      }
  }
};

inline int zm_pick_nseg(int wgs_per_seg, int D, int cap, const char* env_name) {
  int best = 1;
  double best_cost = 1e30;
  for (int n = 1; n <= min(D, cap); ++n) {
    const int len = cds_ceil_div(D, n);
    const int n_eff = cds_ceil_div(D, len);
    const double cost = (double)cds_ceil_div(wgs_per_seg * n_eff, 256) * (len + 1.5);
    if (cost < best_cost - 1e-9) { best_cost = cost; best = n; }
  }
  const int nseg_e = cds_env_int(env_name, 0);
  return nseg_e > 0 ? min(nseg_e, D) : best;
}

}
```

### include/cds_mvsnet_hip.h

```cpp
#ifndef CDS_MVSNET_HIP_H
#define CDS_MVSNET_HIP_H

#ifdef __cplusplus
extern "C" {
#endif

#define CDS_EINVAL (-1000)
#define CDS_MAX_VIEWS 8
#define CDS_MAX_IMAGES 16
#define CDS_STAGE_STATE_WORDS 2080

#define CDS_ACT_NONE 0
#define CDS_ACT_RELU 1
#define CDS_ACT_LEAKY01 2
#define CDS_ACT_SIGMOID 3
#define CDS_ACT_ACCUM 16
#define CDS_ACT_TANH 4

#define CDS_AGG_ACCUMULATE 1
#define CDS_AGG_NORMALIZE 2
#define CDS_AGG_CHANNELS_LAST 4
#define CDS_AGG_FAST_POSITIONS 8
#define CDS_WARP_FAST_POSITIONS CDS_AGG_FAST_POSITIONS

int cds_version(void);

int cds_chw_to_hwc_f32(const float* src_chw, float* dst_hwc, int C, int h, int w, void* stream);

int cds_stage_inputs_f32(const float* const* ref_feas, const float* const* src_feas, const float* const* ref_nc,
                         const float* const* ref_ncsum, const float* const* src_ncsum, float* ref_chw_out, float* src_hwc_out,
                         float* ref_nc_out, float* nc_mean_out, float* state, int V, int C, int h, int w, void* stream);

int cds_homo_warp_f32(const float* src_hwc, const float* mat, const float* hyp, float* out,
                      int C, int D, int h, int w, int hyp_per_pixel, void* stream);

int cds_warp_entropy_f32(const float* ref_chw, const float* src_hwc, const float* mats,
                         const float* hyp, float* entropy, int V, int C, int D, int h, int w,
                         int hyp_per_pixel, void* stream);
int cds_warp_entropy_flags_f32(const float* ref_chw, const float* src_hwc, const float* mats,
                               const float* hyp, float* entropy, int V, int C, int D, int h, int w,
                               int hyp_per_pixel, int flags, void* stream);

int cds_warp_aggregate_f32(const float* ref_chw, const float* src_hwc, const float* vis_w,
                           const float* mats, const float* hyp, float* volume, float* vis_sum,
                           int V, int C, int D, int h, int w, int hyp_per_pixel, int flags,
                           void* stream);

int cds_warp_entropy_window_f32(const float* ref_chw, const float* src_hwc, const float* mats, const float* hyp,
                                float* entropy, int V, int C, int D, int h, int w, int hs, int y_off, int flags, void* stream);
int cds_warp_aggregate_window_f32(const float* ref_chw, const float* src_hwc, const float* vis_w, const float* mats,
                                  const float* hyp, float* volume, float* vis_sum, int V, int C, int D, int h, int w, int hs,
                                  int y_off, int flags, void* stream);

int cds_warp_aggregate_bwd_f32(const float* ref_chw, const float* src_hwc, const float* vis_w,
                               const float* mats, const float* hyp, const float* grad_volume,
                               float* grad_ref, float* grad_src_hwc, float* grad_vis, int V, int C, int D,
                               int h, int w, int hyp_per_pixel, void* stream);
int cds_volume_finish_f32(const float* volume_sum, const float* gt_sum, const float* vis, int V, int C, int D, int hw, float* volume,
                          float* feat_distance, void* stream);
int cds_volume_finish_bwd_f32(const float* g_volume, const float* g_feat_distance, const float* volume_sum, const float* gt_sum,
                              const float* vis, int V, int C, int D, int hw, float* g_volume_sum, float* g_gt_sum, float* g_vis,
                              float* scratch, void* stream);

int cds_volume_normalize_f32(float* volume, const float* vis_sum, int C, int D, int hw, void* stream);

int cds_volume_normalize_cl_f32(float* volume, const float* vis_sum, int C, int D, int hw, void* stream);

int cds_softargmin_conf_f32(const float* prob_pre, const float* hyp, float* depth, float* conf,
                            float* prob, int D, int h, int w, int hyp_per_pixel, void* stream);

int cds_depth_hypotheses_f32(const float* prev_depth, float* out, int D, int hp, int wp, int H, int W,
                             int scale, const float* interval, const float* depth_range, void* stream);

int cds_depth_planes_f32(float* out, int D, int h, int w, const float* depth_range, void* stream);

int cds_conv3d_k3_f32(const float* x, const float* weight, const float* bias, const float* skip,
                      float* out, int Cin, int Cout, int D, int H, int W, int stride, int act,
                      void* stream);

int cds_conv3d_k3_cl_f32(const float* x, const float* weight_cl, const float* bias, const float* skip,
                         float* out, int Cin, int Cout, int D, int H, int W, int act, void* stream);

#define CDS_SBF_PAIR 101
int cds_conv3d_sbf_f32(const float* x, const void* weight_split, const float* bias, const float* skip, float* out,
                       int Cin, int Cout, int D, int H, int W, int stride, int act, void* stream);
int cds_conv3d_sf16_f32(const float* x, const void* weight_split, const float* bias, float* out, int Cin, int Cout, int D, int H, int W,
                        int stride, int act, const float* in_bound, float w_inv_scale, float* out_bound, void* stream);


int cds_deconv3d_sbf_f32(const float* x, const void* weight_split, const float* bias, const float* skip, float* out,
                         int Cin, int Cout, int D, int H, int W, int act, int out_planar, void* stream);

int cds_deconv3d_zm_f32(const float* x, const void* weight_cls, const float* bias, const float* skip, float* out,
                        int Cin, int Cout, int D, int H, int W, int act, void* stream);
int cds_deconv3d_sf16_f32(const float* x, const void* weight_split, const float* bias, const float* skip, float* out, int Cin, int Cout,
                          int D, int H, int W, int act, const float* in_bound, float w_inv_scale, float* out_bound, void* stream);
int cds_deconv3d_zm_sf16_f32(const float* x, const void* weight_cls, const float* bias, const float* skip, float* out, int Cin, int Cout,
                             int D, int H, int W, int act, const float* in_bound, float w_inv_scale, float* out_bound, void* stream);


int cds_deconv_prob_zm_f32(const float* x, const void* weight_split, const float* bias, const float* skip,
                           const float* prob_table, float* out, int D, int H, int W, void* stream);
int cds_deconv_prob_zm_sf16_f32(const float* x, const void* weight_split, const float* bias, const float* skip, const float* prob_table,
                                float* out, int D, int H, int W, const float* in_bound, float w_inv_scale, void* stream);
int cds_deconv_prob_zm_sf16_mfma_f32(const float* x, const void* weight_split, const float* bias, const float* skip,
                                     const float* prob_table, const void* prob_mfma, float* out, int D, int H, int W,
                                     const float* in_bound, float w_inv_scale, const float* skip_bound, float y_gain, float p_inv_scale,
                                     void* stream);


int cds_deconv3d_k3s2_f32(const float* x, const float* weight, const float* bias, const float* skip,
                          float* out, int Cin, int Cout, int D, int H, int W, int act, void* stream);

int cds_conv2d_f32(const float* x, const float* weight, const float* bias, float* out, int N, int Cin,
                   int Cout, int H, int W, int k, int stride, int pad, int act, void* stream);
int cds_conv2d_affine_f32(const float* x, const float* in_affine, const float* weight, const float* bias, float* out,
                          int N, int Cin, int Cout, int H, int W, int k, int stride, int pad, int act, void* stream);

int cds_conv2d_k3_c16_f32(const float* x, const float* weight_cl, const float* bias, const float* head_w,
                          const float* head_b, float* out, int N, int H, int W, int act, void* stream);

int cds_dynconv_branches_sbf_f32(const float* x, const float* in_affine, const void* weight_split, const float* bias,
                                 float* out, int N, int Cin, int Co3, int H, int W, const int* ksizes, int nb, void* stream);

int cds_dynconv_fused_sbf_f32(const float* x, const float* in_affine, const void* weight_split, const float* bias,
                              const float* w1, const float* b1, const float* w2, const float* epipoles,
                              float temperature, float* out, float* norm_curv, double* partial, int N, int Cin, int Cout,
                              int H, int W, const int* ksizes, int nb, void* stream);
int cds_dynconv_fused_parts(int H, int W);

int cds_conv2d_k3_relu_sbf_f32(const float* x, const void* weight_split, const float* bias, const float* head_w,
                               const float* head_b, float* out, int N, int Cin, int H, int W, void* stream);

int cds_fpn_stats_parts(int H, int W);
int cds_conv2d_fpn_f32(const float* coarse, const float* coarse_affine, const float* skip, const float* skip_affine,
                       const float* weight, float* out, float* partial, int N, int Ca, int Cb, int Cout, int H, int W,
                       void* stream);

int cds_dynconv_blend_f32(const float* branches, const float* w1, const float* b1, const float* w2,
                          const float* epipoles, float temperature, float* out, float* norm_curv,
                          int N, int K, int Cout, int H, int W, void* stream);
int cds_dynconv_blend_shared_f32(const float* branches, const float* w1, const float* b1, const float* w2,
                                 const float* epipoles, float temperature, float* out, float* norm_curv, int N,
                                 int K, int Cout, int H, int W, int n_shared, void* stream);

int cds_blend_stats_parts(int H, int W);
int cds_dynconv_blend_stats_f32(const float* branches, const float* w1, const float* b1, const float* w2,
                                const float* epipoles, float temperature, float* out, float* norm_curv,
                                float* partial, int N, int K, int Cout, int H, int W, int n_shared, void* stream);
int cds_instnorm_reduce_f32(const float* partial, int parts, float* stats, float* affine, int N, int C, int H, int W,
                            float slope, void* stream);
int cds_instnorm_apply_f32(const float* x, const float* stats, float* out, int N, int C, int H, int W, int act,
                           int out_hwc, void* stream);

int cds_instnorm_act_f32(const float* x, float* out, float* stats, int N, int C, int H, int W, int act,
                         int out_hwc, void* stream);
int cds_instnorm_affine_f32(const float* x, float* affine, float* stats, int N, int C, int H, int W, float slope,
                            void* stream);

int cds_debug_poison_lds(unsigned pattern);

int cds_dynconv_cl_parts(int H, int W);
int cds_dynconv_cl_f32(const float* x, const float* in_affine, const void* weight_split, const float* bias, const float* w1,
                       const float* b1, const float* w2, const float* epipoles, float temperature, float* out,
                       float* norm_curv, double* partial, int N, int C, int H, int W, const int* ksizes, int nb, void* stream);
int cds_dynconv_cl_sf16_f32(const float* x, const float* in_affine, const void* weight_split, const float* bias, const float* w1,
                            const float* b1, const float* w2, const float* epipoles, float temperature, float* out, float* norm_curv,
                            double* partial, int N, int C, int H, int W, const int* ksizes, int nb, float x_bound, float w_inv_scale,
                            void* stream);

int cds_conv00_cl_f32(const float* x, const void* weight_split, const float* bias, const float* w1, const float* b1, const float* w2,
                      const float* epipoles, float temperature, float* out, float* norm_curv, double* partial, int N, int n_shared,
                      int H, int W, void* stream);
int cds_conv00_cl_sf16_f32(const float* x, const void* weight_split, const float* bias, const float* w1, const float* b1, const float* w2,
                           const float* epipoles, float temperature, float* out, float* norm_curv, double* partial, int N, int n_shared,
                           int H, int W, const float* in_bound, float w_inv_scale, void* stream);

int cds_blend_cl_parts(int H, int W);
int cds_dynconv_blend_cl_f32(const float* branches, const float* w1, const float* b1, const float* w2, const float* epipoles,
                             float temperature, float* out, float* norm_curv, double* partial, int N, int K, int Cout, int H, int W,
                             int n_shared, void* stream);
int cds_conv2d_k3s2_cl_f32(const float* x, const float* in_affine, const float* weight, float* out, int N, int Cin, int Cout, int H,
                           int W, void* stream);
int cds_conv2d_k3s2_cl_sf16_f32(const float* x, const float* in_affine, const void* weight_split, float* out, int N, int Cin, int Cout,
                                int H, int W, float x_bound, float w_inv_scale, void* stream);

int cds_fpn_cl_parts(int H, int W);
int cds_conv2d_fpn_cl_f32(const float* coarse, const float* coarse_affine, const float* skip, const float* skip_affine,
                          const float* weight, float* out, double* partial, int N, int Ca, int Cb, int Cout, int H, int W,
                          void* stream);
int cds_vis_layer1_cl_f32(const float* entropy, const float* ref_nc, const float* weight, const float* bias, float* out, int V, int H,
                          int W, void* stream);
int cds_conv2d_k3_relu_cl_f32(const float* x, const void* weight_split, const float* bias, const float* head_w, const float* head_b,
                              float* out, int N, int Cin, int H, int W, void* stream);
int cds_vis_cnn_rm_f32(const float* entropy, const float* ref_nc, const float* w0, const float* b0, const void* ws1, const float* b1,
                       const void* ws2, const float* b2, const float* head_w, const float* head_b, float* out, int V, int H, int W,
                       void* stream);
int cds_instnorm_stats_cl_parts(int H, int W);
int cds_instnorm_stats_cl_f32(const float* x, double* partial, int N, int C, int H, int W, void* stream);
int cds_instnorm_apply_cl_f32(const float* x, const double* stats, float* out_cl, float* out_chw, int N, int C, int H, int W, int act,
                              int n_chw, int cl_from, void* stream);

int cds_depth_fusion_f32(const float* ref_depth, const float* ref_conf, const float* src_depths,
                         const float* src_confs, const float* cams, float* fused, float* mask, float* points,
                         float* view_masks, int V, int h, int w, const float* prob_thresh_host,
                         float dist_thresh, float depth_thresh, float view_thresh, void* stream);

int cds_depth_fusion_dynamic_f32(const float* ref_depth, const float* ref_conf, const float* src_depths,
                                 const float* src_confs, const float* cams, float* fused, float* mask, float* points,
                                 unsigned char* admit, unsigned char* levels, int V, int h, int w,
                                 const float* prob_thresh_host, float dist_base, float rel_base, int n_min, int n_max,
                                 void* stream);

int cds_depth_normals_f32(const float* depth, const unsigned char* valid, const float* cam_host, int h, int w, int radius,
                          float jump, int min_pts, float* normals, unsigned char* ok, void* stream);

int cds_voxel_merge_f32(const float* points, const unsigned* colors, const float* normals, long long n, const long long* perm,
                        const int* start, long long n_voxels, float* out_points, unsigned* out_colors, float* out_normals,
                        int* out_counts, void* stream);

#define CDS_TSDF_MAX_CHUNK 32
#define CDS_TSDF_MAX_CELLS (1 << 26)
int cds_tsdf_integrate_f32(const int* keys, long long n_blocks, const double* frame_host, const int* dims_host, double trunc,
                           const float* depths, const unsigned char* masks, const unsigned char* images, const double* cams,
                           int n_views, int h, int w, float* sum, int* n, int* nc, int* rgb, void* stream);
int cds_tsdf_classify(const int* keys, const int* table, long long n_blocks, const double* frame_host, const int* dims_host,
                      const float* sum, const int* n, int min_weight, unsigned char* vmask, unsigned char* tcount,
                      int* block_vertices, int* block_faces, void* stream);
int cds_tsdf_emit(const int* keys, const int* table, long long n_blocks, const double* frame_host, const int* dims_host,
                  const float* sum, const int* n, const int* nc, const int* rgb, const unsigned char* vmask,
                  const unsigned char* tcount, const int* block_vstart, const int* block_tstart, long long n_vertices,
                  long long n_faces, int* vstart, float* vertices, unsigned char* colors, int* faces, void* stream);

int cds_tsdf_view_weights(const float* depth, const unsigned char* mask, const float* normals, const unsigned char* ok,
                          const float* conf, const float* cam_host, int h, int w, unsigned char* weights, void* stream);
int cds_tsdf_integrate_w_f32(const int* keys, long long n_blocks, const double* frame_host, const int* dims_host, double trunc,
                             const float* depths, const unsigned char* masks, const unsigned char* images, const double* cams,
                             int n_views, int h, int w, float* sum, int* n, int* nc, int* rgb, const unsigned char* weights,
                             int interp, float jump, int* wn, void* stream);

#define CDS_RASTER_CAM 24
#define CDS_RASTER_MAX_CHUNK 32
#define CDS_RASTER_MAX_LIST (1ll << 30)
int cds_raster_project(const float* vertices, long long n_vertices, const double* cams, int n_views, int* xy, double* xc,
                       void* stream);
int cds_raster_faces(const int* faces, long long n_faces, long long n_vertices, const double* cams, int n_views, const int* xy,
                     const double* xc, int h, int w, long long large_px, unsigned long long* keys, unsigned char* large,
                     void* stream);
int cds_raster_large(const long long* list, long long n_list, const int* faces, long long n_faces, long long n_vertices,
                     const double* cams, int n_views, const int* xy, const double* xc, int h, int w, unsigned long long* keys,
                     void* stream);
int cds_raster_resolve(const unsigned long long* keys, const int* faces, long long n_faces, long long n_vertices,
                       const double* cams, int n_views, const double* xc, const unsigned char* colors, int h, int w, float* depth,
                       int* face, unsigned char* front, unsigned char* valid, unsigned char* image, void* stream);

#define CDS_MESH_CC_MAX_ROUNDS 64
int cds_mesh_cc_init(int* parent, long long n_vertices, void* stream);
int cds_mesh_cc_hook(const int* faces, long long n_faces, long long n_vertices, int* parent, int* changed, void* stream);
int cds_mesh_cc_jump(int* parent, long long n_vertices, void* stream);
int cds_mesh_cc_count(const int* faces, long long n_faces, long long n_vertices, const int* label, int* count, void* stream);
int cds_mesh_cc_mark(const int* faces, long long n_faces, long long n_vertices, const int* label, const unsigned char* keep,
                     unsigned char* face_keep, unsigned char* vertex_keep, void* stream);
int cds_mesh_cc_gather(const float* vertices, const unsigned char* colors, const int* faces, long long n_vertices,
                       long long n_faces, const unsigned char* vertex_keep, const int* vertex_new, const unsigned char* face_keep,
                       const int* face_new, long long out_vertices, long long out_faces, float* vertices_out,
                       unsigned char* colors_out, int* faces_out, void* stream);

int cds_mesh_simplify_faces(const int* faces, long long n_faces, long long n_vertices, const int* cluster, long long n_clusters,
                            int* face_clusters, unsigned char* collapsed, int* identity, void* stream);
int cds_mesh_simplify_quadric_f32(const float* vertices, long long n_vertices, const int* faces, long long n_faces,
                                  const long long* perm, const int* start, const long long* inc, const int* inc_start,
                                  long long n_clusters, float cell, float* out_positions, unsigned char* out_fallback,
                                  void* stream);
int cds_mesh_simplify_mark(const int* face_clusters, const unsigned char* face_keep, long long n_faces, long long n_clusters,
                           unsigned char* cluster_keep, void* stream);
int cds_mesh_simplify_gather(const float* positions, const unsigned* colors, long long n_clusters,
                             const unsigned char* cluster_keep, const int* cluster_new, const int* face_clusters, long long n_faces,
                             const unsigned char* face_keep, const int* face_new, long long out_vertices, long long out_faces,
                             float* vertices_out, unsigned char* colors_out, int* faces_out, void* stream);

#define CDS_MESH_ADJ_SMALL 64
#define CDS_MESH_ADJ_BOUNDARY 1
#define CDS_MESH_ADJ_ISOLATED 2
int cds_mesh_adj_small(void);
int cds_mesh_adj_count(const int* faces, long long n_faces, long long n_vertices, int* count, void* stream);
int cds_mesh_adj_fill(const int* faces, long long n_faces, long long n_vertices, const int* start, int* cursor, int* nbr,
                      long long n_entries, void* stream);
int cds_mesh_adj_finish(long long n_vertices, const int* start, int* nbr, long long n_entries, int* deg, unsigned char* flags,
                        void* stream);
int cds_mesh_smooth_step_f32(const float* in, float* out, long long n_vertices, const int* start, const int* deg, const int* nbr,
                             double factor, void* stream);
int cds_mesh_smooth_limit_f32(const float* original, float* vertices, long long n_vertices, double max_move, double* move2_out,
                              unsigned char* clamped_out, void* stream);

#define CDS_MESH_FILL_MAX_EDGES 4096
int cds_mesh_fill_max_edges(void);
int cds_mesh_fill_keys(const int* faces, long long n_faces, long long n_vertices, long long* keys, void* stream);
int cds_mesh_fill_borders(const long long* keys, long long n_keys, long long n_vertices, int* out, int* in, int* next, int* prev,
                          void* stream);
int cds_mesh_fill_init(long long n_vertices, const int* out, const int* in, int* next, int* prev, unsigned char* regular,
                       int* label_a, int* jump_a, int* label_b, int* jump_b, void* stream);
int cds_mesh_fill_double(const int* list, long long n_list, long long n_vertices, const int* label_in, const int* jump_in,
                         int* label_out, int* jump_out, void* stream);
int cds_mesh_fill_walk(const float* vertices, const unsigned char* colors, long long n_vertices, const int* next,
                       const unsigned char* regular, const int* label, const int* list, long long n_list, int max_edges, int* edges,
                       float* centre, unsigned char* centre_color, void* stream);
int cds_mesh_fill_emit(const int* next, const unsigned char* regular, long long n_vertices, long long n_faces, const int* list,
                       long long n_list, int max_edges, const int* edges, const long long* vertex_at, const long long* face_at,
                       const float* centre, const unsigned char* centre_color, long long new_vertices, long long new_faces,
                       float* vertices_out, unsigned char* colors_out, int* faces_out, void* stream);

#define CDS_MESH_SAMPLE_MAX_N 32768
int cds_mesh_sample_max_n(void);
int cds_mesh_sample_count(const float* vertices, long long n_vertices, const int* faces, long long n_faces, double spacing,
                          int* out_n, long long* out_n2, void* stream);
int cds_mesh_sample_emit(const float* vertices, const unsigned char* colors, long long n_vertices, const int* faces,
                         long long n_faces, const int* n, const long long* offsets, long long n_points, float* out_points,
                         unsigned char* out_colors, int* out_face, void* stream);

#define CDS_TEXTURE_MAX_CELL 4096
#define CDS_TEXTURE_MAX_SIZE 32768
#define CDS_TEXTURE_MAX_UNITS (1ll << 26)
int cds_texture_votes(const int* face, const unsigned char* valid, int n_views, int h, int w, long long n_faces, int* votes,
                      int runs, void* stream);
int cds_texture_best(const int* votes, long long n_faces, int n_views, int view0, unsigned long long* key, void* stream);
int cds_texture_cells(const float* vertices, long long n_vertices, const int* faces, long long n_faces, const double* cams,
                      int n_views, const unsigned long long* key, long long min_px, double scale, int max_cell, int* view,
                      int* cell, void* stream);
int cds_texture_place(const long long* order, const long long* starts, long long n_faces, long long total, int max_cell, int* cell,
                      int* uv, void* stream);
int cds_texture_fill(const float* vertices, const unsigned char* colors, long long n_vertices, const int* faces, long long n_faces,
                     const double* cams, const unsigned char* images, long long image_bytes, const long long* views, int n_views,
                     const int* view, const int* cell, const long long* order, const long long* starts, long long total,
                     int max_cell, int atlas_h, int atlas_w, unsigned char* atlas, int per_unit, void* stream);

#define CDS_TEXTURE_LEVEL_MAX_VIEWS 512
#define CDS_TEXTURE_LEVEL_OMEGA 0.75
int cds_texture_level_samples(const float* vertices, long long n_vertices, const double* cams, const unsigned char* images,
                              long long image_bytes, const long long* views, int n_views, const long long* node_key,
                              long long n_nodes, double* sample, unsigned char* ok, void* stream);
int cds_texture_level_pairs(const double* sample, const unsigned char* ok, const long long* node_key, const int* span,
                            long long n_nodes, int n_views, long long* table, void* stream);
int cds_texture_level_step(const double* sample, const unsigned char* ok, const int* span, const long long* corner_start,
                           const long long* corner_list, long long n_list, const int* corner_node, long long n_nodes,
                           long long n_faces, int n_views, double lambda, const double* g_in, double* g_out, void* stream);
int cds_texture_fill_level(const float* vertices, const unsigned char* colors, long long n_vertices, const int* faces,
                           long long n_faces, const double* cams, const unsigned char* images, long long image_bytes,
                           const long long* views, int n_views, const int* view, const int* cell, const long long* order,
                           const long long* starts, long long total, int max_cell, int atlas_h, int atlas_w, unsigned char* atlas,
                           int per_unit, const int* corner_node, const double* g, long long n_nodes, void* stream);

#define CDS_PHOTO_TILE 16
#define CDS_PHOTO_RECORD 8
#define CDS_PHOTO_SCORES_WS_WORDS(n_views, h, w) \
  ((long long)(n_views) * (((h) + CDS_PHOTO_TILE - 1) / CDS_PHOTO_TILE) * (((w) + CDS_PHOTO_TILE - 1) / CDS_PHOTO_TILE) * CDS_PHOTO_RECORD)
int cds_photo_shade(const float* vertices, long long n_vertices, const int* faces, long long n_faces, const int* uv,
                    const unsigned char* atlas, int atlas_h, int atlas_w, const double* cams, int n_views, const int* face, int h,
                    int w, unsigned char* image, void* stream);
int cds_photo_scores(const unsigned char* a, const unsigned char* b, const unsigned char* mask, const double* g, int n_views, int h,
                     int w, long long* ws, long long ws_words, long long* counts, double* ssim_sum, double* ssim_map, void* stream);

int cds_curvature_stats_f32(const float* a, const float* b, const float* c, float* nc_sum, float* nc_abs, int n,
                            void* stream);
int cds_curvature_stats_bwd_f32(const float* a, const float* b, const float* c, const float* g_sum, const float* g_abs, float* ga,
                                float* gb, float* gc, int n, void* stream);
int cds_pair_mean_f32(const float* x, float* out, int V, int n, void* stream);
int cds_view_mean_f32(const float* x, float* out, int V, int n, void* stream);

int cds_depth_affine_f32(const float* depth, float* out, int n, const float* depth_range, void* stream);
int cds_deconv2d_k3s2_f32(const float* x, const float* weight, const float* bias, float* out, int Cin, int Cout,
                          int H, int W, int act, void* stream);
int cds_refine_finish_f32(const float* d_norm, const float* res, float* out, int h, int w, const float* depth_range,
                          void* stream);

int cds_bn3d_stats_f32(const float* x, double* sums, int B, int C, long long V, void* stream);
int cds_bn3d_norm_f32(const float* y, const double* sums, const float* gamma, const float* beta, double n, double eps, float momentum,
                      float* running_mean, float* running_var, const float* skip, float* out, float* scale, float* shift, double* mean,
                      double* invstd, int B, int C, long long V, int relu, void* stream);
int cds_bn3d_bwd_reduce_f32(const float* dout, const float* y, const float* scale, const float* shift, double* sums, int B,
                            int C, long long V, int relu, void* stream);
int cds_bn3d_bwd_norm_f32(const float* dout, const float* y, const float* scale, const float* shift, const double* sums,
                          const double* mean, const double* invstd, double n, float* dy, float* dgamma, float* dbeta, int B, int C,
                          long long V, int relu, void* stream);
int cds_conv3d_wgrad_f32(const float* g, const float* xin, float* dw, int B, int Ca, int Cb, int Do, int Ho, int Wo, int Di,
                         int Hi, int Wi, int stride, void* stream);

int cds_bn3d_norm_bound_f32(const float* y, const double* sums, const float* gamma, const float* beta, double n, double eps,
                            float momentum, float* running_mean, float* running_var, const float* skip, float* out, float* scale,
                            float* shift, double* mean, double* invstd, int B, int C, long long V, int relu, float* out_bound,
                            void* stream);
int cds_bn3d_bwd_norm_bound_f32(const float* dout, const float* y, const float* scale, const float* shift, const double* sums,
                                const double* mean, const double* invstd, double n, float* dy, float* dgamma, float* dbeta, int B, int C,
                                long long V, int relu, float* dy_bound, void* stream);
int cds_absmax_bound_f32(const float* x, long long n, float* bound, void* stream);
int cds_sf16_pack_conv3d_f32(const float* w, void* fwd, void* dgrad, float* w_inv, int A, int B, int mode, void* stream);
int cds_conv3d_k3_sf16_f32(const float* x, const void* wpk, const float* w_inv, const float* x_bound, float* y, int B, int C, int M,
                           int Di, int Hi, int Wi, int mode, void* stream);
int cds_conv3d_wgrad_sf16_f32(const float* g, const float* xin, const float* g_bound, const float* x_bound, float* dw, int B, int Ca,
                              int Cb, int Do, int Ho, int Wo, int Di, int Hi, int Wi, int stride, void* stream);

int cds_conv2d_wgrad_f32(const float* g, const float* x, float* dw, int N, int Co, int Cin, int Ho, int Wo, int H, int W, int k,
                         int stride, int pad, void* stream);
int cds_conv2d_dgrad_s2_f32(const float* g, const float* w, float* gx, int N, int Co, int Cin, int Ho, int Wo, int H, int W,
                            void* stream);
int cds_instnorm_bwd_f32(const float* gz, const float* y, const double* stats, double* sums, float* gy, int N, int C, int H, int W,
                         int act, int scratch_zeroed, void* stream);
int cds_dynconv_bn_stats_f32(const float* branches, const float* epipoles, const float* w1, double* mom, float* mean, float* rstd,
                             float* running_mean, float* running_var, int N, int G, int K, int Cout, int H, int W, float eps,
                             float momentum, int use_batch, int scratch_zeroed, void* stream);
int cds_dynconv_blend_train_f32(const float* branches, const float* epipoles, const float* w1, const float* w2, const float* gamma,
                                const float* beta, const float* mean, const float* rstd, float temperature, float* out,
                                float* norm_curv, int N, int G, int K, int Cout, int H, int W, void* stream);
int cds_dynconv_blend_bwd_f32(const float* branches, const float* epipoles, const float* w1, const float* w2, const float* gamma,
                              const float* beta, const float* mean, const float* rstd, float temperature, const float* gy,
                              const float* gnc, float* gbr, double* sums, double* dw1, int N, int G, int K, int Cout, int H, int W,
                              int use_batch, int scratch_zeroed, void* stream);
int cds_f32_to_bf16(const float* src, unsigned short* dst, long long n, void* stream);
int cds_instnorm_act_b16_f32(const float* y, unsigned short* y16, float* out32, unsigned short* out16, double* stats, int N, int C,
                             int H, int W, int act, int strict, void* stream);
int cds_conv2d_wgrad_xb16_f32(const float* g, const unsigned short* x, float* dw, int N, int Co, int Cin, int Ho, int Wo, int H, int W,
                              int k, int stride, int pad, void* stream);
int cds_instnorm_bwd_yb16_f32(const float* gz, const unsigned short* y, const unsigned short* z16, const double* stats, double* sums,
                              float* gy, int N, int C, int H, int W, int act, int scratch_zeroed, void* stream);
int cds_dynconv_bn_stats_b16_f32(const unsigned short* branches, const float* epipoles, const float* w1, double* mom, float* mean,
                                 float* rstd, float* running_mean, float* running_var, int N, int G, int K, int Cout, int H, int W,
                                 float eps, float momentum, int use_batch, int scratch_zeroed, void* stream);
int cds_dynconv_blend_train_b16_f32(const unsigned short* branches, const float* epipoles, const float* w1, const float* w2,
                                    const float* gamma, const float* beta, const float* mean, const float* rstd, float temperature,
                                    float* out, float* norm_curv, int N, int G, int K, int Cout, int H, int W, void* stream);
int cds_dynconv_blend_bwd_b16_f32(const unsigned short* branches, const float* epipoles, const float* w1, const float* w2,
                                  const float* gamma, const float* beta, const float* mean, const float* rstd, float temperature,
                                  const float* gy, const float* gnc, float* gbr, double* sums, double* dw1, int N, int G, int K,
                                  int Cout, int H, int W, int use_batch, int scratch_zeroed, void* stream);
int cds_pack_conv2d_f32(const float* wa, const float* wb, float* fwd, float* dgrad, int Ca, int Cb, int Cin, int k, void* stream);
int cds_pack_conv3d_f32(const float* w, float* fwd, float* dgrad, int A, int B, int mode, void* stream);
int cds_softargmin_bwd_f32(const float* prob_pre, const float* hyp, const float* gdepth, float* gpre, int D, int h, int w,
                           int hyp_per_pixel, void* stream);
int cds_dynconv_bwd_finish_f32(const double* sums, const double* dw1, int G, int K, float* out, void* stream);

int cds_loss_records(long long elements);
int cds_loss_stage_f32(const float* depth, const float* gt, const float* mask, const float* norm_curv, const float* dist,
                       const float* target, const float* interval, int B, int hw, int Dp, double* recA, double* recB, void* stream);
int cds_loss_final_f32(const double* const* recA, const double* const* recB, const long long* pixels, const int* Dp, const float* weight,
                       const int* has_curv, int n_stages, float* total, float* depth_loss, double* scalars, void* stream);
int cds_loss_stage_bwd_f32(const float* depth, const float* gt, const float* mask, const float* dist, const float* target,
                           const float* interval, const float* gtotal, const double* scalars, float weight, int B, int hw, int Dp,
                           float* gdepth, float* gnc, float* gdist, void* stream);
int cds_feat_target_f32(const float* hyp, const float* gt, const float* di, float scale, float thresh, int B, int D, int hw,
                        float* target, void* stream);

int cds_bn_running_update_f32(const float* batch_mean, const float* batch_var, const float* group_weights, float keep, int G, int C,
                              float* running_mean, float* running_var, void* stream);

int cds_grid_hash_log2_slots(long long n_keys);
int cds_grid_keys_f32(const float* points, long long n, const float* frame_host, long long* keys, void* stream);
int cds_grid_hash_build(const long long* keys, long long n_keys, long long n_fine, long long* table_keys, int* table_vals,
                        int log2_slots, void* stream);
int cds_nn_query_f32(const float* query, const long long* order, long long m, const float* pts, const int* cell_start,
                     const long long* cell_keys, const int* coarse_start, const long long* table_keys, const int* table_vals,
                     int log2_slots, const float* frame_host, float max_dist, float* dist, void* stream);
int cds_thin_round_f32(const float* pts, const int* cell_start, long long n, const long long* table_keys, const int* table_vals,
                       int log2_slots, const float* frame_host, float min_dist, unsigned char* state, int* undecided,
                       void* stream);

#define CDS_ICP_SUMS 18
#define CDS_ICP_MAX_GROUPS 1024
#define CDS_ICP_WS_DOUBLES (CDS_ICP_MAX_GROUPS * CDS_ICP_SUMS)
#define CDS_CROP_MAX_VERTICES 256
int cds_transform_points_f32(const float* points, long long n, const double* T, float* out, void* stream);
int cds_nn_index_f32(const float* query, const long long* order, long long m, const float* pts, const int* cell_start,
                     const long long* cell_keys, const int* coarse_start, const long long* table_keys, const int* table_vals,
                     int log2_slots, const float* frame_host, float max_dist, float* dist, int* index, void* stream);
int cds_icp_sums_f64(const float* source, const long long* order, long long m, const double* T, const float* pts,
                     const int* cell_start, const long long* cell_keys, const int* coarse_start, const long long* table_keys,
                     const int* table_vals, int log2_slots, const float* frame_host, float max_dist, double* ws,
                     long long ws_doubles, double* out, int* index, float* dist, void* stream);
int cds_voxel_mean_f32(const float* points, long long n, const long long* perm, const int* start, long long n_voxels, float* out,
                       void* stream);
int cds_polygon_crop_f32(const float* points, long long n, const double* polygon, int P, int axis, double axis_min,
                         double axis_max, unsigned char* keep, void* stream);

#define CDS_KNN_MAX_K 64
#define CDS_STAT_CHUNK 4096
int cds_knn_mean_f64(const float* query, const long long* order, long long m, const float* pts, const int* cell_start,
                     const long long* cell_keys, const int* coarse_start, const long long* table_keys, const int* table_vals,
                     int log2_slots, const float* frame_host, int k, float max_dist, double* mean, float* kth, void* stream);
int cds_knn_mean_wg_f64(const float* query, const long long* order, long long m, const float* pts, const int* cell_start,
                        const long long* cell_keys, const int* coarse_start, const long long* table_keys, const int* table_vals,
                        int log2_slots, const float* frame_host, int k, float max_dist, double* mean, float* kth, int threads,
                        void* stream);
int cds_radius_count_f32(const float* query, const long long* order, long long m, const float* pts, const int* cell_start,
                         const long long* cell_keys, const int* coarse_start, const long long* table_keys, const int* table_vals,
                         int log2_slots, const float* frame_host, float radius, int cap, int* count, void* stream);
int cds_outlier_stats_f64(const double* x, long long n, double* ws, long long ws_doubles, double* out, void* stream);

#define CDS_RANSAC_RECORD 15
#define CDS_RANSAC_MIN_SAMPLE 3
#define CDS_RANSAC_MAX_SAMPLE 8
int cds_ransac_similarity_f64(const double* src, const double* dst, long long n, long long hypotheses, int k, double threshold,
                              unsigned long long seed, double* ws, long long ws_doubles, double* out, int* count, double* err2,
                              void* stream);

int cds_gipuma_tiles(long long n);
int cds_gipuma_prob_filter_f32(const float* depths, const float* confs, const unsigned char* rgb8, int V, int h, int w,
                               const float* prob_thresh_host, float* depth_out, unsigned* rgb_out, void* stream);
int cds_gipuma_fuse_view_f32(const float* depths, const unsigned* rgb, const float* views, const float* fb, int r, int V, int h,
                             int w, float depth_min, float depth_max, float disp_thresh, int num_consistent, unsigned char* used,
                             unsigned char* emit, unsigned* records, void* stream);
int cds_gipuma_scan(const unsigned char* emit, int tiles, int* tile_count, int* tile_off, int* total, void* stream);
int cds_gipuma_compact_f32(const unsigned char* emit, const unsigned* records, const int* tile_off, int tiles, int hw,
                           float* points, unsigned* colors, int* ref_view, void* stream);

#define CDS_COLMAP_SCORE_QUANTUM_LOG2 80
#define CDS_COLMAP_SCORE_MAX_LIMBS 28
int cds_colmap_score_quantum_log2(void);
int cds_colmap_score_limbs(double theta0, double sigma1, double sigma2);
int cds_colmap_pair_scores_f64(const long long* pair_off, const long long* ptr, const int* img, const int* cnt,
                               const double* xyz, const double* centres, long long P, long long T, int N, double theta0,
                               double sigma1, double sigma2, int limbs, long long* acc, void* stream);
int cds_colmap_obs_depth_f64(const int* obs_img, const long long* obs_pt, const double* xyz, const double* zrow, long long n,
                             double* z, void* stream);
int cds_colmap_depth_ranges_f64(const double* z_sorted, const long long* obs_ptr, const int* num_min, const int* num_max,
                                int N, double* out, void* stream);

#define CDS_DEPTH_METRICS_MAX_T 8
#define CDS_DEPTH_METRICS_MAX_GROUPS 1024
#define CDS_DEPTH_METRICS_WS_DOUBLES(B) \
  ((long long)(B) * (CDS_DEPTH_METRICS_MAX_GROUPS / (B) < 1 ? 1 : CDS_DEPTH_METRICS_MAX_GROUPS / (B)) * (3 * CDS_DEPTH_METRICS_MAX_T + 5))
int cds_depth_metrics_f32(const float* est, const float* gt, const float* mask, const float* thr, float cap, int B, long long hw, int T,
                          double* ws, long long ws_doubles, double* out, void* stream);
int cds_gt_pyramid_f32(const float* src, const unsigned char* mask_src, int mask_thresh, int Hs, int Ws, const int* rows, const int* cols,
                       int h, int w, int levels, float* depth_out, float* mask_out, void* stream);

int cds_image_batch_u8(const unsigned char* src, int n, int Hs, int Ws, const int* rows, const int* cols, int h, int w, float* out,
                       void* stream);

int cds_eval_views_u8(const unsigned char* src, int V, int Hs, int Ws, const int* row0, const int* row1, const float* fy, const int* col0,
                      const int* col1, const float* fx, int h, int w, float* out, void* stream);
int cds_eval_outputs_f32(const float* c1, int H1, int W1, const float* c2, int H2, int W2, const float* c3, int H3, int W3,
                         const float* img, int Hi, int Wi, const int* tab, int h, int w, float* conf3, unsigned char* img_u8,
                         void* stream);

#ifdef __cplusplus
}
#endif
#endif
```

Baseline: 192.5 depth-maps/s.

## Add balanced persistent work partitioning across CUs for z-march conv/deconv kernels

Adds a balanced scheduling mode for the z-marching 3D conv, deconv and deconv-prob kernels. It launches about one workgroup per CU, and each workgroup walks an equal share of the flattened column×depth-stage space as a sequence of column pieces. The mode is used only when a host-side cost model predicts it beats the uniform segment split by a margin. The aim is to remove the wave-quantization tail imbalance. The cost is extra pipeline restarts per piece, added syncthreads, and more template instantiations.

```diff
diff --git a/cds_mvsnet_amd/_lib.py b/cds_mvsnet_amd/_lib.py
--- a/cds_mvsnet_amd/_lib.py
+++ b/cds_mvsnet_amd/_lib.py
@@ -58,6 +58,9 @@
     "cds_deconv_prob_zm_sf16_f32": [P, P, P, P, P, P, I, I, I, P, F, P],
     "cds_deconv_prob_zm_sf16_mfma_f32": [P, P, P, P, P, P, P, I, I, I, P, F, P, F, F, P],
     "cds_deconv3d_zm_f32": [P, P, P, P, P, I, I, I, I, I, I, P],
+    "cds_zm_partition": [I, I, I, I, I, I, P],
+    "cds_zm_partition_all": [I, I, I, I, I, I, P],
+    "cds_zm_plan": [I, I, I, I, I, I, I, P],
     "cds_deconv3d_k3s2_f32": [P, P, P, P, P, I, I, I, I, I, I, P],
     "cds_conv2d_f32": [P, P, P, P, I, I, I, I, I, I, I, I, I, P],
     "cds_conv2d_affine_f32": [P, P, P, P, P, I, I, I, I, I, I, I, I, I, P],
diff --git a/cds_mvsnet_amd/csrc/conv3d_zmg.hip b/cds_mvsnet_amd/csrc/conv3d_zmg.hip
--- a/cds_mvsnet_amd/csrc/conv3d_zmg.hip
+++ b/cds_mvsnet_amd/csrc/conv3d_zmg.hip
@@ -1,7 +1,10 @@
 #include <stdlib.h>
+
+#include <type_traits>
 
 #include "cds_common.hpp"
 #include "sbf_common.hpp"
+#include "zm_common.hpp"
 
 namespace {
 
@@ -9,7 +12,7 @@
 
 struct ZGDefaults {
   static constexpr int S = 1, RD = 1, MB = 1, TXO = 16, TYO = 8, G = 1, NG = 1, CW = 8, RPW = 1, YS = 1, PF = 1;
-  static constexpr bool PAIR = false, F16 = false, P32 = false;
+  static constexpr bool PAIR = false, F16 = false, P32 = false, BALANCED = true;
 };
 template <class P>
 struct ZgF16 : P {
@@ -49,10 +52,11 @@
 };
 struct ZgConv5F16 : ZgF16<ZGDefaults> {
   static constexpr int S = 2, RD = 4, MB = 4, TYO = 2, RPW = 2;
-  static constexpr bool P32 = true;
+  static constexpr bool P32 = true, BALANCED = false;
 };
 struct ZgConv6F16 : ZgF16<ZGDefaults> {
   static constexpr int RD = 8, MB = 4, TYO = 2, RPW = 2, YS = 2;
+  static constexpr bool BALANCED = false;
 };
 
 template <class P>
@@ -100,7 +104,14 @@
   static constexpr int PT = PW * 64, PPT = (NITEM + PT - 1) / PT;
 };
 
-template <class Cfg>
+struct ZmgNoWalk {
+  __device__ __forceinline__ ZmgNoWalk(int, int, int, int) {}
+  __device__ __forceinline__ bool empty() const { return false; }
+  __device__ __forceinline__ ZmColumn column(int) const { return {0, 0, 0, 0}; }
+  __device__ __forceinline__ bool next_piece() { return false; }
+};
+
+template <class Cfg, bool BAL>
 __global__ __launch_bounds__(Cfg::THREADS, 1) void conv3d_zmg_kernel(const float* __restrict__ x, const uint4* __restrict__ wsp,
                                                                   const float* __restrict__ bias, float* __restrict__ out, int Cout,
                                                                   int D, int H, int W, int Do, int Ho, int Wo, int act,
@@ -116,15 +127,27 @@
   const int tid = threadIdx.x;
   const int lane = tid & 63;
   const int wave = __builtin_amdgcn_readfirstlane(tid >> 6);
-  const int nseg = (Do + zseg - 1) / zseg;
-  int unit = cds_xcd_remap(blockIdx.x, gridDim.x);
-  const int seg = unit % nseg;
-  unit /= nseg;
-  const int tx_i = unit % tiles_x, ty_i = unit / tiles_x;
-  const int z0 = seg * zseg, z1 = min(Do, z0 + zseg);
-  const int nstages = (z1 - z0 + G - 1) / G;
-  const int gx0 = tx_i * Cfg::TXO * S - 1, gy0 = ty_i * Cfg::TYO * S - 1;
-  const int zin0 = S * z0 - 1;
+  std::conditional_t<BAL, ZmWalk<true>, ZmgNoWalk> walk(tiles_x * tiles_y, (Do + G - 1) / G, 0, ZM_MINLEN_ZMG);
+  if (BAL && walk.empty()) return;
+  int tx_i, ty_i, z0, z1, nstages, gx0, gy0, zin0;
+  auto set_piece = [&] {
+    if constexpr (BAL) {
+      const ZmColumn zc = walk.column(tiles_x);
+      tx_i = zc.tx_i, ty_i = zc.ty_i, z0 = zc.a0 * G, z1 = min(Do, zc.a1 * G);
+    } else {
+      const int nseg = (Do + zseg - 1) / zseg;
+      int unit = cds_xcd_remap(blockIdx.x, gridDim.x);
+      const int seg = unit % nseg;
+      unit /= nseg;
+      tx_i = unit % tiles_x, ty_i = unit / tiles_x;
+      z0 = seg * zseg, z1 = min(Do, z0 + zseg);
+    }
+    nstages = (z1 - z0 + G - 1) / G;
+    gx0 = tx_i * Cfg::TXO * S - 1, gy0 = ty_i * Cfg::TYO * S - 1;
+    zin0 = S * z0 - 1;
+    return true;
+  };
+  set_piece();
 
   if (wave >= Cfg::CW) {
 #ifndef CDS_ZMG_PPRIO
@@ -133,6 +156,7 @@
     __builtin_amdgcn_s_setprio(CDS_ZMG_PPRIO);
     constexpr int PT = Cfg::PT, PPT = Cfg::PPT;
     const int ptid = tid - Cfg::CW * 64;
+    do {
     int s_pl[PPT], s_dst[PPT];
     long long s_off[PPT];
     unsigned okmask = 0;
@@ -207,6 +231,7 @@
       }
       __syncthreads();
     }
+    } while (BAL && walk.next_piece() && set_piece());
     return;
   }
 
@@ -238,21 +263,25 @@
   float amax = 0.f;
   const int co = PAIR ? 4 * (g & 1) : mbg * 16 + 4 * g;
   const float4 bv = (bias && co < Cout) ? *reinterpret_cast<const float4*>(bias + co) : make_float4(0.f, 0.f, 0.f, 0.f);
+  const int xl = PAIR ? 2 * j + (g >> 1) : j;
+  do {
   constexpr int XW = PAIR ? 32 : 16;
+  constexpr bool UBASE = Cfg::P32 || BAL;
   const int oy0 = ty_i * Cfg::TYO + part * Cfg::ROWS;
-  const int ox0 = tx_i * Cfg::TXO + (PAIR ? 2 * j + (g >> 1) : j);
+  const int ox0 = tx_i * Cfg::TXO + xl;
+  const int x_left = Wo - tx_i * Cfg::TXO;
   float* const obase = out + ((size_t)((size_t)z0 * Ho + oy0) * Wo + ox0) * Cout + co;
   float* const obase_u = out + ((size_t)((size_t)z0 * Ho + oy0) * Wo + tx_i * Cfg::TXO) * Cout;
-  const unsigned olane = (unsigned)((ox0 - tx_i * Cfg::TXO) * Cout + co);
+  const unsigned olane = BAL ? (unsigned)(xl * Cout + co) : (unsigned)((ox0 - tx_i * Cfg::TXO) * Cout + co);
   auto out_ptr = [&](int pl, int r, int xt) -> float* {
     const size_t o = ((size_t)((size_t)pl * Ho + r) * Wo + xt * XW) * Cout;
-    return Cfg::P32 ? obase_u + o + olane : obase + o;
+    return UBASE ? obase_u + o + olane : obase + o;
   };
   bool lane_ok[Cfg::XT];
 #pragma unroll
-  for (int xt = 0; xt < Cfg::XT; ++xt) lane_ok[xt] = ox0 + xt * XW < Wo && co < Cout;
+  for (int xt = 0; xt < Cfg::XT; ++xt) lane_ok[xt] = (BAL ? xl + xt * XW < x_left : ox0 + xt * XW < Wo) && co < Cout;
   auto in_x_ct = [&](int xt) { return lane_ok[xt]; };
-  auto in_x_rt = [&](int xt) { return ox0 + xt * XW < Wo && co < Cout; };
+  auto in_x_rt = [&](int xt) { return (BAL ? xl + xt * XW < x_left : ox0 + xt * XW < Wo) && co < Cout; };
   auto store_tile = [&](int n, int st, const f32x4& a, auto in_x) {
     const int i = n % G, rx = n / G, xt = rx % Cfg::XT, r = rx / Cfg::XT;
     if (z0 + st * G + i >= z1 || oy0 + r >= Ho) return;
@@ -379,11 +408,13 @@
     __syncthreads();
   }
   if (Cfg::KSPL >= 2 || late) finish(nstages - 1);
+  } while (BAL && walk.next_piece() && set_piece());
   if (F16) sf16_publish_bound(amax, out_bound);
 }
 
-inline int zmg_pick_nseg(int cols, int Do, int G) {
+inline int zmg_pick_nseg(int cols, int Do, int G, double* cost_out = nullptr) {
   const int nseg_env = cds_env_int("CDS_ZMG_NSEG", 0);
+  if (cost_out) *cost_out = -1.0;
   if (nseg_env > 0) return nseg_env;
   const int stages = cds_ceil_div(Do, G);
   int best = 1;
@@ -394,7 +425,21 @@
     const double cost = (double)cds_ceil_div(cols * cds_ceil_div(stages, per), 256) * (per + 2.5);
     if (cost < best_cost - 1e-9) { best_cost = cost; best = n; }
   }
+  if (cost_out) *cost_out = best_cost;
   return best;
+}
+
+struct ZmgPlan {
+  int nseg, nwg;
+  bool balanced;
+  double ucost, bcost;
+};
+inline ZmgPlan zmg_plan(int cols, int ys, int Do, int G, int ncu, int balance) {
+  ZmgPlan p;
+  p.nseg = zmg_pick_nseg(cols * ys, Do, G, &p.ucost);
+  p.nwg = max(1, ncu / ys);
+  p.balanced = zm_choose_balanced(balance, p.ucost, cols, cds_ceil_div(Do, G), p.nwg, ZM_MINLEN_ZMG, 2.5, &p.bcost);
+  return p;
 }
 
 template <class P>
@@ -404,15 +449,27 @@
   constexpr int S = Cfg::S;
   const int Do = (D - 1) / S + 1, Ho = (H - 1) / S + 1, Wo = (W - 1) / S + 1;
   const int tx = cds_ceil_div(Wo, Cfg::TXO), ty = cds_ceil_div(Ho, Cfg::TYO);
-  int nseg = zmg_pick_nseg(tx * ty * Cfg::YS, Do, Cfg::G);
+  const ZmgPlan plan = zmg_plan(tx * ty, Cfg::YS, Do, Cfg::G, zm_ncu(), zm_balance_knob());
+  int nseg = plan.nseg;
   const int zseg = cds_ceil_div(cds_ceil_div(Do, nseg), Cfg::G) * Cfg::G;
   nseg = cds_ceil_div(Do, zseg);
   if (min_wgs > 0 && tx * ty * nseg * Cfg::YS < min_wgs) return CDS_ZMG_UNSUPPORTED;
-  return cds_launch_lds<conv3d_zmg_kernel<Cfg>>(Cfg::LDSB, dim3(tx * ty * nseg, Cfg::YS), dim3(Cfg::THREADS), Cfg::LDSB, st, x,
-                                                reinterpret_cast<const uint4*>(wsp), b, out, Cout, D, H, W, Do, Ho, Wo, act, tx, ty, zseg,
-                                                in_bound, w_inv, out_bound);
-}
-
+  if constexpr (P::BALANCED)
+    if (plan.balanced)
+      return cds_launch_lds<conv3d_zmg_kernel<Cfg, true>>(Cfg::LDSB, dim3(plan.nwg, Cfg::YS), dim3(Cfg::THREADS), Cfg::LDSB, st, x,
+                                                          reinterpret_cast<const uint4*>(wsp), b, out, Cout, D, H, W, Do, Ho, Wo, act, tx,
+                                                          ty, zseg, in_bound, w_inv, out_bound);
+  return cds_launch_lds<conv3d_zmg_kernel<Cfg, false>>(Cfg::LDSB, dim3(tx * ty * nseg, Cfg::YS), dim3(Cfg::THREADS), Cfg::LDSB, st, x,
+                                                       reinterpret_cast<const uint4*>(wsp), b, out, Cout, D, H, W, Do, Ho, Wo, act, tx, ty,
+                                                       zseg, in_bound, w_inv, out_bound);
+}
+
+}
+
+int cds_zmg_plan(int cols, int ys, int Do, int G, int ncu, int balance, int* nseg, double* ucost, double* bcost) {
+  const ZmgPlan p = zmg_plan(cols, ys, Do, G, ncu, balance);
+  *nseg = p.nseg, *ucost = p.ucost, *bcost = p.bcost;
+  return p.balanced;
 }
 
 int cds_conv3d_zmg_dispatch(const float* x, const void* wsp, const float* bias, float* out, int Cin, int Cout, int D, int H, int W,
diff --git a/cds_mvsnet_amd/csrc/deconv3d_zm.hip b/cds_mvsnet_amd/csrc/deconv3d_zm.hip
--- a/cds_mvsnet_amd/csrc/deconv3d_zm.hip
+++ b/cds_mvsnet_amd/csrc/deconv3d_zm.hip
@@ -36,7 +36,7 @@
   }
 }
 
-template <int ROUNDS, bool F16>
+template <int ROUNDS, bool F16, bool BAL>
 __global__ __launch_bounds__((DZC<ROUNDS>::THREADS), 3) void deconv3d_zm_kernel(
     const float* __restrict__ x, const uint4* __restrict__ wcls, const float* __restrict__ bias, const float* __restrict__ skip,
     float* __restrict__ out, int D, int H, int W, int tiles_x, int ncols, int seg_len, int act, const float* __restrict__ in_bound,
@@ -50,14 +50,15 @@
   const int tid = threadIdx.x;
   const int lane = tid & 63;
   const int wave = __builtin_amdgcn_readfirstlane(tid >> 6);
-  const ZmColumn zc = zm_column(tiles_x, ncols, seg_len, D);
-  const int a0 = zc.a0, a1 = zc.a1;
-  if (a0 >= a1) return;
-  const int X0 = zc.tx_i * C::TX, Y0 = zc.ty_i * C::TY;
+  ZmWalk<BAL> walk(ncols, D, seg_len, ZM_MINLEN_CELL);
+  if (walk.empty()) return;
   const int Ho = 2 * H, Wo = 2 * W;
 
   if (wave >= C::CW) {
-    dzm_produce<C, F16>(x, lds, tid - C::CW * 64, X0, Y0, D, H, W, a0, a1, xs);
+    do {
+      const ZmColumn zc = walk.column(tiles_x);
+      dzm_produce<C, F16>(x, lds, tid - C::CW * 64, zc.tx_i * C::TX, zc.ty_i * C::TY, D, H, W, zc.a0, zc.a1, xs);
+    } while (BAL && walk.next_piece());
     return;
   }
 
@@ -77,10 +78,14 @@
   }
   const float4 bv = bias ? *reinterpret_cast<const float4*>(bias + 4 * g) : make_float4(0.f, 0.f, 0.f, 0.f);
   const int b_off = (((g >> 1) * C::IXP) + j + (g & 1)) * POSB;
+  const size_t zstride = (size_t)Ho * Wo * Cout;
+  float amax = 0.f;
+  do {
+  const ZmColumn zc = walk.column(tiles_x);
+  const int a0 = zc.a0, a1 = zc.a1;
+  const int X0 = zc.tx_i * C::TX, Y0 = zc.ty_i * C::TY;
   const int xv = 2 * (X0 + j) + px;
   const bool x_ok = X0 + j < W;
-  const size_t zstride = (size_t)Ho * Wo * Cout;
-  float amax = 0.f;
   __syncthreads();
   for (int a = a0; a < a1; ++a) {
     const unsigned char* lo = lds + (a % C::NSLOT) * C::SLOTB + b_off;
@@ -131,11 +136,13 @@
     }
     __syncthreads();
   }
+  } while (BAL && walk.next_piece());
   if (F16) sf16_publish_bound(amax, out_bound);
 }
 
 
 constexpr int DZM64_W1L = 2;
+template <bool BAL>
 __global__ __launch_bounds__((DZC<8, 4>::THREADS), 3) void deconv3d_zm64_kernel(
     const float* __restrict__ x, const uint4* __restrict__ wsp, const float* __restrict__ bias, const float* __restrict__ skip,
     float* __restrict__ out, int D, int H, int W, int tiles_x, int ncols, int seg_len, int act, const float* __restrict__ in_bound,
@@ -148,15 +155,16 @@
   const int tid = threadIdx.x;
   const int lane = tid & 63;
   const int wave = __builtin_amdgcn_readfirstlane(tid >> 6);
-  const ZmColumn zc = zm_column(tiles_x, ncols, seg_len, D);
-  const int a0 = zc.a0, a1 = zc.a1;
-  if (a0 >= a1) return;
+  ZmWalk<BAL> walk(ncols, D, seg_len, ZM_MINLEN_CELL);
+  if (walk.empty()) return;
   const int mbtot = gridDim.y, mb0 = blockIdx.y;
-  const int X0 = zc.tx_i * C::TX, Y0 = zc.ty_i * C::TY;
   const int Ho = 2 * H, Wo = 2 * W;
 
   if (wave >= C::CW) {
-    dzm_produce<C, true>(x, lds, tid - C::CW * 64, X0, Y0, D, H, W, a0, a1, xs);
+    do {
+      const ZmColumn zc = walk.column(tiles_x);
+      dzm_produce<C, true>(x, lds, tid - C::CW * 64, zc.tx_i * C::TX, zc.ty_i * C::TY, D, H, W, zc.a0, zc.a1, xs);
+    } while (BAL && walk.next_piece());
     return;
   }
 
@@ -183,11 +191,15 @@
   const bool live = g < (1 + pz) * ny * nx;
   const int dz = live ? g / (ny * nx) : 0, dy = live ? (g / nx) % ny : 0, dx = live ? g % nx : 0;
   const int b_off = ((dy * C::IXP) + j + dx) * POSB;
+  const size_t zstride = (size_t)Ho * Wo * Cout;
+  float amax = 0.f;
+  do {
+  const ZmColumn zc = walk.column(tiles_x);
+  const int a0 = zc.a0, a1 = zc.a1;
+  const int X0 = zc.tx_i * C::TX, Y0 = zc.ty_i * C::TY;
   const int xv = 2 * (X0 + j) + px;
   const bool x_ok = X0 + j < W;
-  const size_t zstride = (size_t)Ho * Wo * Cout;
   const int nrows = min(C::TY, H - Y0);
-  float amax = 0.f;
   __syncthreads();
   for (int a = a0; a < a1; ++a) {
     const unsigned char* p0 = lds + (a % C::NSLOT) * C::SLOTB + b_off;
@@ -235,6 +247,7 @@
     }
     __syncthreads();
   }
+  } while (BAL && walk.next_piece());
   sf16_publish_bound(amax, out_bound);
 }
 
@@ -248,12 +261,18 @@
   using C = DZC<8, 4>;
   const int tiles_x = cds_ceil_div(W, C::TX), tiles_y = cds_ceil_div(H, C::TY);
   const int ncols = tiles_x * tiles_y;
-  const int seg_len = cds_ceil_div(D, zm_pick_nseg(ncols * 2, D, 24, "CDS_DZM_NSEG"));
+  double ucost;
+  const int seg_len = cds_ceil_div(D, zm_pick_nseg(ncols * 2, D, 24, "CDS_DZM_NSEG", &ucost));
   const int nseg = cds_ceil_div(D, seg_len);
   if (deep == 1 && ncols * nseg * 2 < 256) return CDS_ZMG_UNSUPPORTED;
-  return cds_launch_lds<deconv3d_zm64_kernel>(160 * 1024, dim3(ncols * nseg, 2), dim3(C::THREADS), C::LDS + DZM64_W1L * 2 * 1024, st, x,
-                                              reinterpret_cast<const uint4*>(wsp), bias, skip, out, D, H, W, tiles_x, ncols, seg_len, act,
-                                              in_bound, w_inv, out_bound);
+  const int nwg = max(1, zm_ncu() / 2);
+  const bool bal = zm_choose_balanced(zm_balance_knob(), ucost, ncols, D, nwg, ZM_MINLEN_CELL, 1.5);
+  auto launch = [&](auto b) {
+    return cds_launch_lds<deconv3d_zm64_kernel<decltype(b)::value>>(
+        160 * 1024, dim3(b ? nwg : ncols * nseg, 2), dim3(C::THREADS), C::LDS + DZM64_W1L * 2 * 1024, st, x,
+        reinterpret_cast<const uint4*>(wsp), bias, skip, out, D, H, W, tiles_x, ncols, seg_len, act, in_bound, w_inv, out_bound);
+  };
+  return bal ? launch(std::true_type()) : launch(std::false_type());
 }
 
 static int dzm_entry(const float* x, const void* weight_cls, const float* bias, const float* skip, float* out, int Cin, int Cout, int D,
@@ -264,14 +283,61 @@
   hipStream_t st = (hipStream_t)stream;
   const int tiles_x = cds_ceil_div(W, C::TX), tiles_y = cds_ceil_div(H, C::TY);
   const int ncols = tiles_x * tiles_y;
-  const int seg_len = cds_ceil_div(D, zm_pick_nseg(ncols, D, 24, "CDS_DZM_NSEG"));
+  double ucost;
+  const int seg_len = cds_ceil_div(D, zm_pick_nseg(ncols, D, 24, "CDS_DZM_NSEG", &ucost));
   const int nseg = cds_ceil_div(D, seg_len);
-  auto launch = [&](auto f16) {
-    return cds_launch_lds<deconv3d_zm_kernel<4, decltype(f16)::value>>(160 * 1024, dim3(ncols * nseg), dim3(C::THREADS), C::LDS, st, x,
-                                                                       reinterpret_cast<const uint4*>(weight_cls), bias, skip, out, D, H, W,
-                                                                       tiles_x, ncols, seg_len, act, in_bound, w_inv, out_bound);
+  const int nwg = zm_ncu();
+  const bool bal = zm_choose_balanced(zm_balance_knob(), ucost, ncols, D, nwg, ZM_MINLEN_CELL, 1.5);
+  auto launch = [&](auto f16, auto b) {
+    return cds_launch_lds<deconv3d_zm_kernel<4, decltype(f16)::value, decltype(b)::value>>(
+        160 * 1024, dim3(b ? nwg : ncols * nseg), dim3(C::THREADS), C::LDS, st, x, reinterpret_cast<const uint4*>(weight_cls), bias, skip,
+        out, D, H, W, tiles_x, ncols, seg_len, act, in_bound, w_inv, out_bound);
   };
-  return in_bound ? launch(std::true_type()) : launch(std::false_type());
+  if (bal) return in_bound ? launch(std::true_type(), std::true_type()) : launch(std::false_type(), std::true_type());
+  return in_bound ? launch(std::true_type(), std::false_type()) : launch(std::false_type(), std::false_type());
+}
+
+extern "C" int cds_zm_partition(int cols, int planes, int unit, int nwg, int wg, int min_len, int* out) {
+  if (cols < 1 || planes < 1 || unit < 1 || nwg < 1 || wg < 0 || wg >= nwg || min_len < 1 || !out) return CDS_EINVAL;
+  ZmPiece pc[ZM_MAX_PIECES];
+  const int n = zm_partition(cols, cds_ceil_div(planes, unit), nwg, wg, min_len, pc);
+  for (int i = 0; i < min(n, ZM_MAX_PIECES); ++i) {
+    out[3 * i] = pc[i].col;
+    out[3 * i + 1] = pc[i].s0 * unit;
+    out[3 * i + 2] = min(planes, pc[i].s1 * unit);
+  }
+  return n;
+}
+extern "C" int cds_zm_partition_all(int cols, int planes, int unit, int nwg, int min_len, int cap, int* out) {
+  if (cols < 1 || planes < 1 || unit < 1 || nwg < 1 || min_len < 1 || cap < 1 || !out) return CDS_EINVAL;
+  const int stages = cds_ceil_div(planes, unit);
+  for (int wg = 0; wg < nwg; ++wg) {
+    int* o = out + (size_t)wg * (1 + 3 * cap);
+    const ZmRange r = zm_range(cols, stages, nwg, wg, min_len);
+    int n = 0;
+    for (int pos = r.lo; pos < r.hi; ++n) {
+      const ZmPiece p = zm_piece_at(pos, r.hi, stages);
+      if (n < cap) o[1 + 3 * n] = p.col, o[2 + 3 * n] = p.s0 * unit, o[3 + 3 * n] = min(planes, p.s1 * unit);
+      pos = p.col * stages + p.s1;
+    }
+    o[0] = n;
+  }
+  return 0;
+}
+int cds_zmg_plan(int cols, int ys, int Do, int G, int ncu, int balance, int* nseg, double* ucost, double* bcost);
+extern "C" int cds_zm_plan(int family, int cols, int planes, int unit, int ys, int ncu, int balance, int* out) {
+  if (family < 0 || family > 2 || cols < 1 || planes < 1 || unit < 1 || ys < 1 || ncu < 1 || !out) return CDS_EINVAL;
+  int nseg = 0, bal = 0;
+  double ucost = 0, bcost = 0;
+  if (family == 0) {
+    bal = cds_zmg_plan(cols, ys, planes, unit, ncu, balance, &nseg, &ucost, &bcost);
+  } else {
+    nseg = zm_pick_nseg(cols * ys, planes, family == 1 ? 24 : 16, "", &ucost);
+    bal = zm_choose_balanced(balance, ucost, cols, planes, max(1, ncu / ys), ZM_MINLEN_CELL, 1.5, &bcost,
+                             family == 2 ? ZM_BALANCE_MARGIN_TAIL : ZM_BALANCE_MARGIN);
+  }
+  out[0] = bal, out[1] = nseg, out[2] = (int)lrint(ucost * 1000), out[3] = (int)lrint(bcost * 1000);
+  return 0;
 }
 
 extern "C" int cds_deconv3d_zm_f32(const float* x, const void* weight_cls, const float* bias, const float* skip, float* out,
diff --git a/cds_mvsnet_amd/csrc/deconv_prob_zm.hip b/cds_mvsnet_amd/csrc/deconv_prob_zm.hip
--- a/cds_mvsnet_amd/csrc/deconv_prob_zm.hip
+++ b/cds_mvsnet_amd/csrc/deconv_prob_zm.hip
@@ -43,7 +43,7 @@
     if constexpr (F16) { SF16_TERMS(ACC, 0, C::NT, W, X); }   \
     else { SBF_TERMS(ACC, 0, C::NT, W, X); }                  \
   } while (0)
-template <bool F16, bool MF>
+template <bool F16, bool MF, bool BAL>
 __global__ __launch_bounds__(DPZ::THREADS, 3) void deconv_prob_zm_kernel(
     const float* __restrict__ x, const uint4* __restrict__ wsp, const float* __restrict__ bias, const float* __restrict__ skip,
     const float* __restrict__ pw, float* __restrict__ out, int D, int H, int W, int tiles_x, int ncols, int seg_len,
@@ -64,13 +64,15 @@
   const int tid = threadIdx.x;
   const int lane = tid & 63;
   const int wave = __builtin_amdgcn_readfirstlane(tid >> 6);
-  const ZmColumn zc = zm_column(tiles_x, ncols, seg_len, D);
-  const int tx_i = zc.tx_i, ty_i = zc.ty_i, a0 = zc.a0, a1 = zc.a1;
-  if (a0 >= a1) return;
-  const int X0 = tx_i * C::CXR - 1, Y0 = ty_i * C::CYR - 1;
+  ZmWalk<BAL> walk(ncols, D, seg_len, ZM_MINLEN_CELL);
+  if (walk.empty()) return;
   const int Do = 2 * D, Ho = 2 * H, Wo = 2 * W;
-  const int qs = a0 > 0 ? 2 * a0 - 1 : 0;
-  const int qe = min(Do - 1, 2 * a1);
+#define DPZ_PIECE()                                                                                               \
+  const ZmColumn zc = walk.column(tiles_x);                                                                       \
+  const int tx_i = zc.tx_i, ty_i = zc.ty_i, a0 = zc.a0, a1 = zc.a1;                                               \
+  const int X0 = tx_i * C::CXR - 1, Y0 = ty_i * C::CYR - 1;                              \
+  const int qs = a0 > 0 ? 2 * a0 - 1 : 0;                                   \
+  const int qe = min(Do - 1, 2 * a1);                                                               \
   const int te = 2 * a1 + 1;
   {
     uint4* wdst = reinterpret_cast<uint4*>(lds);
@@ -81,7 +83,6 @@
     __builtin_amdgcn_s_setprio(2);
     const int ptid = tid - C::CW * 64;
     ZmCellStage<C, C::PW * 64, F16, true> stage;
-    stage.init(ptid, X0, Y0, H, W);
     auto issue = [&](int plane) { stage.issue(x, plane, D, H, W); };
     auto deposit = [&](int plane) { stage.deposit(inring + (plane & 1) * C::SLOTB, xs); };
     if constexpr (MF) {
@@ -92,23 +93,15 @@
       for (int r = 0; r < 3; ++r)
 #pragma unroll
         for (int ky = 0; ky < 3; ++ky) wa[r][ky].u = pwm[(r * 3 + ky) * 64 + lane];
-      const int oy0 = ty_i * 2 * C::CYR + C::PR * rg;
       int b_off[C::MT];
 #pragma unroll
       for (int t = 0; t < C::MT; ++t) {
         const int xl = C::MSTEP * t + n;
         b_off[t] = (g & 1) * C::YTERMB + (xl & 1) * C::YPARB + (((xl >> 1) ^ ((xl & 1) << 3)) << 4);
       }
-      const int ox0 = tx_i * 2 * C::CXR + n - 2;
       const bool st_ok = g < 3 && n >= 2 && n <= 13;
-      const unsigned st_lane = st_ok ? oy0 * Wo + ox0 : 0;
-      const int st_lim = st_ok ? Wo - ox0 : 0;
       const float inv = p_inv / ys;
       float A[C::MT][C::PR];
-#pragma unroll
-      for (int t = 0; t < C::MT; ++t)
-#pragma unroll
-        for (int r = 0; r < C::PR; ++r) A[t][r] = 0.f;
       const int yrow0 = (C::PR * rg + 1) * C::YROWB;
       auto load_b = [&](BV (&b)[C::PR + 2], const unsigned char* yb, int t) {
 #pragma unroll
@@ -137,6 +130,17 @@
           }
         }
       };
+      do {
+      DPZ_PIECE()
+      stage.init(ptid, X0, Y0, H, W);
+      const int oy0 = ty_i * 2 * C::CYR + C::PR * rg;
+      const int ox0 = tx_i * 2 * C::CXR + n - 2;
+      const unsigned st_lane = st_ok ? oy0 * Wo + ox0 : 0;
+      const int st_lim = st_ok ? Wo - ox0 : 0;
+#pragma unroll
+      for (int t = 0; t < C::MT; ++t)
+#pragma unroll
+        for (int r = 0; r < C::PR; ++r) A[t][r] = 0.f;
       const int ap = qs >> 1;
       issue(ap);
       deposit(ap);
@@ -171,21 +175,13 @@
           for (int r = 0; r < C::PR; ++r) A[tt][r] = own ? 0.f : A[tt][r];
         __syncthreads();
       }
+      } while (BAL && walk.next_piece());
       return;
     }
     const int c = ptid & 63, rg = ptid >> 6;
-    const int ox = tx_i * 2 * C::CXR + c;
-    const int oy0 = ty_i * 2 * C::CYR + C::PR * rg;
-    const bool lane_ok = c < 2 * C::CXR && ox < Wo;
     const int yoff = (C::PR * rg + 1) * C::YROWB + (c + 1) * 16;
     int st_off[C::PR];
-#pragma unroll
-    for (int r = 0; r < C::PR; ++r) st_off[r] = (lane_ok && oy0 + r < Ho) ? (oy0 + r) * Wo + ox : -1;
     float A[3][C::PR];
-#pragma unroll
-    for (int s = 0; s < 3; ++s)
-#pragma unroll
-      for (int r = 0; r < C::PR; ++r) A[s][r] = 0.f;
     const f32x4* __restrict__ pw4 = reinterpret_cast<const f32x4*>(pw);
     auto load_d = [&](f32x4 (&d)[C::PR + 2], const unsigned char* yb, int b) {
 #pragma unroll
@@ -236,6 +232,18 @@
       DPZ_BATCH(5, d1, wq1, d0, wq0)
 #undef DPZ_BATCH
     };
+    do {
+    DPZ_PIECE()
+    stage.init(ptid, X0, Y0, H, W);
+    const int ox = tx_i * 2 * C::CXR + c;
+    const int oy0 = ty_i * 2 * C::CYR + C::PR * rg;
+    const bool lane_ok = c < 2 * C::CXR && ox < Wo;
+#pragma unroll
+    for (int r = 0; r < C::PR; ++r) st_off[r] = (lane_ok && oy0 + r < Ho) ? (oy0 + r) * Wo + ox : -1;
+#pragma unroll
+    for (int s = 0; s < 3; ++s)
+#pragma unroll
+      for (int r = 0; r < C::PR; ++r) A[s][r] = 0.f;
     const int ap = qs >> 1;
     issue(ap);
     deposit(ap);
@@ -262,6 +270,7 @@
       }
       __syncthreads();
     }
+    } while (BAL && walk.next_piece());
     return;
   }
 
@@ -272,6 +281,8 @@
   const int b_h1 = ((wave + (g >> 1)) * C::IXP + j + (g & 1)) * POSB;
   const int b_h2a = (wave * C::IXP + j + (g & 1)) * POSB;
   const int b_h2b = b_h2a + C::IXP * POSB;
+  do {
+  DPZ_PIECE()
   int sk_off[2][C::NT];
 #pragma unroll
   for (int py = 0; py < 2; ++py)
@@ -389,6 +400,8 @@
     }
     __syncthreads();
   }
+  } while (BAL && walk.next_piece());
+#undef DPZ_PIECE
 }
 
 }
@@ -402,15 +415,21 @@
   hipStream_t st = (hipStream_t)stream;
   const int tiles_x = cds_ceil_div(W, C::CXR), tiles_y = cds_ceil_div(H, C::CYR);
   const int ncols = tiles_x * tiles_y;
-  const int seg_len = cds_ceil_div(D, zm_pick_nseg(ncols, D, 16, "CDS_DPZ_NSEG"));
+  double ucost;
+  const int seg_len = cds_ceil_div(D, zm_pick_nseg(ncols, D, 16, "CDS_DPZ_NSEG", &ucost));
   const int nseg = cds_ceil_div(D, seg_len);
-  auto launch = [&](auto f16, auto mf) {
-    return cds_launch_lds<deconv_prob_zm_kernel<decltype(f16)::value, decltype(mf)::value>>(
-        160 * 1024, dim3(ncols * nseg), dim3(C::THREADS), C::LDS, st, x, reinterpret_cast<const uint4*>(weight_split), bias, skip, prob_table,
-        out, D, H, W, tiles_x, ncols, seg_len, in_bound, w_inv, skip_bound, y_gain, p_inv);
-  };
-  if (skip_bound) return launch(std::true_type(), std::true_type());
-  return in_bound ? launch(std::true_type(), std::false_type()) : launch(std::false_type(), std::false_type());
+  const int nwg = zm_ncu();
+  const bool bal = zm_choose_balanced(zm_balance_knob(), ucost, ncols, D, nwg, ZM_MINLEN_CELL, 1.5, nullptr, ZM_BALANCE_MARGIN_TAIL);
+  auto launch = [&](auto f16, auto mf, auto b) {
+    return cds_launch_lds<deconv_prob_zm_kernel<decltype(f16)::value, decltype(mf)::value, decltype(b)::value>>(
+        160 * 1024, dim3(b ? nwg : ncols * nseg), dim3(C::THREADS), C::LDS, st, x, reinterpret_cast<const uint4*>(weight_split), bias, skip,
+        prob_table, out, D, H, W, tiles_x, ncols, seg_len, in_bound, w_inv, skip_bound, y_gain, p_inv);
+  };
+  auto forms = [&](auto b) {
+    if (skip_bound) return launch(std::true_type(), std::true_type(), b);
+    return in_bound ? launch(std::true_type(), std::false_type(), b) : launch(std::false_type(), std::false_type(), b);
+  };
+  return bal ? forms(std::true_type()) : forms(std::false_type());
 }
 
 extern "C" int cds_deconv_prob_zm_f32(const float* x, const void* weight_split, const float* bias, const float* skip,
diff --git a/cds_mvsnet_amd/csrc/zm_common.hpp b/cds_mvsnet_amd/csrc/zm_common.hpp
--- a/cds_mvsnet_amd/csrc/zm_common.hpp
+++ b/cds_mvsnet_amd/csrc/zm_common.hpp
@@ -6,12 +6,83 @@
 struct ZmColumn {
   int tx_i, ty_i, a0, a1;
 };
-__device__ __forceinline__ ZmColumn zm_column(int tiles_x, int ncols, int seg_len, int D) {
-  const int wg = cds_xcd_remap(blockIdx.x, gridDim.x);
-  const int col = wg % ncols, seg = wg / ncols;
-  const int a0 = seg * seg_len;
-  return {col % tiles_x, col / tiles_x, a0, min(D, a0 + seg_len)};
+
+constexpr int ZM_MAX_PIECES = 8;
+constexpr int ZM_MINLEN_CELL = 3, ZM_MINLEN_ZMG = 4;
+
+struct ZmRange {
+  int lo, hi;
+};
+struct ZmPiece {
+  int col, s0, s1;
+};
+__host__ __device__ inline int zm_snap(long long b, int stages, int q, int min_len) {
+  const long long col = b / stages;
+  int r = (int)(b - col * stages);
+  r = ((r + q / 2) / q) * q;
+  if (r < min_len) r = 0;
+  if (r > 0 && r > stages - min_len) r = stages;
+  return (int)(col * stages + r);
 }
+__host__ __device__ inline ZmRange zm_range(int cols, int stages, int nwg, int wg, int min_len) {
+  const long long T = (long long)cols * stages;
+  const int q = T / nwg >= min_len ? 1 : min_len;
+  return {zm_snap(wg * T / nwg, stages, q, min_len), zm_snap((wg + 1ll) * T / nwg, stages, q, min_len)};
+}
+__host__ __device__ inline ZmPiece zm_piece_at(int pos, int hi, int stages) {
+  const int col = pos / stages, s0 = pos - col * stages;
+  const int rest = hi - col * stages;
+  return {col, s0, rest < stages ? rest : stages};
+}
+__host__ __device__ inline int zm_partition(int cols, int stages, int nwg, int wg, int min_len, ZmPiece* out) {
+  const ZmRange r = zm_range(cols, stages, nwg, wg, min_len);
+  int n = 0;
+  for (int pos = r.lo; pos < r.hi; ++n) {
+    const ZmPiece p = zm_piece_at(pos, r.hi, stages);
+    if (n < ZM_MAX_PIECES) out[n] = p;
+    pos = p.col * stages + p.s1;
+  }
+  return n;
+}
+
+template <bool BAL>
+struct ZmWalk {
+  int col, s0, s1, hi, stages;
+  __device__ __forceinline__ ZmWalk(int cols, int stages_, int seg_len, int min_len) : stages(stages_) {
+    const int wg = cds_xcd_remap(blockIdx.x, gridDim.x);
+    if (BAL) {
+      const ZmRange r = zm_range(cols, stages, gridDim.x, wg, min_len);
+      hi = __builtin_amdgcn_readfirstlane(r.hi);
+      set(__builtin_amdgcn_readfirstlane(r.lo));
+    } else {
+      col = wg % cols;
+      s0 = (wg / cols) * seg_len;
+      s1 = min(stages, s0 + seg_len);
+      hi = 0;
+    }
+  }
+  __device__ __forceinline__ void set(int pos) {
+    if (pos < hi) {
+      const ZmPiece p = zm_piece_at(pos, hi, stages);
+      col = __builtin_amdgcn_readfirstlane(p.col), s0 = __builtin_amdgcn_readfirstlane(p.s0), s1 = __builtin_amdgcn_readfirstlane(p.s1);
+    } else {
+      col = 0, s0 = 0, s1 = 0;
+    }
+  }
+  __device__ __forceinline__ bool empty() const { return s0 >= s1; }
+  __device__ __forceinline__ ZmColumn column(int tiles_x) const {
+    if (!BAL) return {col % tiles_x, col / tiles_x, s0, s1};
+    const int ty_i = __builtin_amdgcn_readfirstlane(col / tiles_x);
+    return {col - ty_i * tiles_x, ty_i, s0, s1};
+  }
+  __device__ __forceinline__ bool next_piece() {
+    const int pos = col * stages + s1;
+    if (pos >= hi) return false;
+    set(pos);
+    __syncthreads();
+    return true;
+  }
+};
 
 template <class C, int NTHR, bool F16, bool LOWHALO>
 struct ZmCellStage {
@@ -54,7 +125,7 @@
   }
 };
 
-inline int zm_pick_nseg(int wgs_per_seg, int D, int cap, const char* env_name) {
+inline int zm_pick_nseg(int wgs_per_seg, int D, int cap, const char* env_name, double* cost_out = nullptr) {
   int best = 1;
   double best_cost = 1e30;
   for (int n = 1; n <= min(D, cap); ++n) {
@@ -64,7 +135,56 @@
     if (cost < best_cost - 1e-9) { best_cost = cost; best = n; }
   }
   const int nseg_e = cds_env_int(env_name, 0);
+  if (cost_out) *cost_out = nseg_e > 0 ? -1.0 : best_cost;
   return nseg_e > 0 ? min(nseg_e, D) : best;
 }
 
+inline int zm_ncu() {
+  const int e = cds_env_int("CDS_ZM_NCU", 0);
+  if (e > 0) return e;
+  static std::atomic<int> cache[64];
+  int d = 0;
+  (void)hipGetDevice(&d);
+  int v = cache[d & 63].load(std::memory_order_relaxed);
+  if (v > 0) return v;
+  if (hipDeviceGetAttribute(&v, hipDeviceAttributeMultiprocessorCount, d) != hipSuccess || v < 1) {
+    (void)hipGetLastError();
+    v = 256;
+  }
+  cache[d & 63].store(v, std::memory_order_relaxed);
+  return v;
 }
+
+inline double zm_balanced_cost(int cols, int stages, int nwg, int min_len, double P, int* max_pieces) {
+  struct Memo { int cols, stages, nwg, min_len, maxp; double P, cost; };
+  thread_local Memo memo[8] = {};
+  thread_local int next = 0;
+  for (const Memo& m : memo)
+    if (m.cols == cols && m.stages == stages && m.nwg == nwg && m.min_len == min_len && m.P == P) { *max_pieces = m.maxp; return m.cost; }
+  double cost = 0;
+  int maxp = 0;
+  for (int wg = 0; wg < nwg; ++wg) {
+    ZmPiece pc[ZM_MAX_PIECES];
+    const ZmRange r = zm_range(cols, stages, nwg, wg, min_len);
+    const int n = zm_partition(cols, stages, nwg, wg, min_len, pc);
+    maxp = max(maxp, n);
+    cost = fmax(cost, (r.hi - r.lo) + P * n);
+  }
+  memo[next] = {cols, stages, nwg, min_len, maxp, P, cost};
+  next = (next + 1) % 8;
+  *max_pieces = maxp;
+  return cost;
+}
+
+constexpr double ZM_BALANCE_MARGIN = 0.02, ZM_BALANCE_MARGIN_TAIL = 0.08;
+inline bool zm_choose_balanced(int balance, double uniform_cost, int cols, int stages, int nwg, int min_len, double P,
+                               double* balanced_cost = nullptr, double margin = ZM_BALANCE_MARGIN) {
+  int maxp = 0;
+  const double bc = zm_balanced_cost(cols, stages, nwg, min_len, P, &maxp);
+  if (balanced_cost) *balanced_cost = bc;
+  if (balance <= 0 || uniform_cost < 0 || maxp > ZM_MAX_PIECES) return false;
+  return balance >= 2 || bc < uniform_cost * (1.0 - margin);
+}
+inline int zm_balance_knob() { return cds_env_int("CDS_ZM_BALANCE", 1); }
+
+}
diff --git a/include/cds_mvsnet_hip.h b/include/cds_mvsnet_hip.h
--- a/include/cds_mvsnet_hip.h
+++ b/include/cds_mvsnet_hip.h
@@ -107,6 +107,10 @@
                                      const float* prob_table, const void* prob_mfma, float* out, int D, int H, int W,
                                      const float* in_bound, float w_inv_scale, const float* skip_bound, float y_gain, float p_inv_scale,
                                      void* stream);
+
+int cds_zm_partition(int cols, int planes, int unit, int nwg, int wg, int min_len, int* out);
+int cds_zm_partition_all(int cols, int planes, int unit, int nwg, int min_len, int cap, int* out);
+int cds_zm_plan(int family, int cols, int planes, int unit, int ys, int ncu, int balance, int* out);
 
 
 int cds_deconv3d_k3s2_f32(const float* x, const float* weight, const float* bias, const float* skip,
```

After: 195.6 depth-maps/s (median of 6 runs). +1.6%, better.
